# Kotstantinovskiy/SonicDiffusionBayesLab

Measured on AMD Instinct MI355X. Metric: 512x512 images/sec at 50 DDIM steps, higher is better.
Workload: dtype bf16; 1 GPU; SD-1.5 512x512 DDIM 50 steps, CFG 7.5, batch=8/GPU (BASELINE configs[1]); global_batch=8, sample_size=64, parallelism=batch-shard x1, weights=SD-1.5-shaped synthetic seed 1234

## Files before the change

include/sd_hip.h:

```cpp
#ifndef SD_HIP_H
#define SD_HIP_H

#ifdef __cplusplus
extern "C" {
#endif

typedef struct sd_unet sd_unet;

typedef struct sd_unet_config {
    int sample_size;
    int in_channels;
    int out_channels;
    int num_levels;
    int block_out_channels[8];
    int layers_per_block;
    int attn_levels[8];
    int cross_attention_dim;
    int num_heads;
    int norm_num_groups;
    float norm_eps;
    int context_len;
    int weight_dtype;
    float fp8_act_scale_norm;
    float fp8_act_scale_ff;
// ... 65 lines not shown
    int vocab_size;
    int hidden_size;
    int num_layers;
    int num_heads;
    int intermediate_size;
    int max_positions;
    float layer_norm_eps;
} sd_clip_config;
typedef struct sd_unet sd_clip;
int sd_clip_create(const sd_clip_config* cfg, sd_clip** out);
int sd_clip_encode(sd_clip* c, void* stream, const int* input_ids, int batch, float* hidden_out, void* workspace,
                   long long workspace_bytes);

typedef struct sd_clip_vision_config {
    int hidden_size;
    int num_layers;
    int num_heads;
    int intermediate_size;
    int image_size;
    int patch_size;
    int projection_dim;
    float layer_norm_eps;
    int hidden_act;
} sd_clip_vision_config;
enum { SD_ACT_QUICK_GELU = 0, SD_ACT_GELU = 1 };
typedef struct sd_unet sd_clip_vision;
int sd_clip_create_projected(const sd_clip_config* cfg, int projection_dim, int eos_token_id, sd_clip** out);
long long sd_clip_text_embeds_workspace_bytes(sd_clip* c, int batch);
int sd_clip_text_embeds(sd_clip* c, void* stream, const int* input_ids, int batch, float* text_embeds, void* workspace,
                        long long workspace_bytes);
int sd_clip_vision_create(const sd_clip_vision_config* cfg, sd_clip_vision** out);
long long sd_clip_vision_workspace_bytes(sd_clip_vision* v, int batch, int height, int width);
int sd_clip_vision_encode(sd_clip_vision* v, void* stream, const unsigned char* images, int batch, int height, int width,
                          float* image_embeds, void* workspace, long long workspace_bytes);
int sd_clip_score(void* stream, const float* image_embeds, const float* text_embeds, int batch, int dim, float* raw,
                  float* score);
int sd_clip_resize_taps(int in_size, int out_size, int first, int count, int* xmin, int* xcnt, int* coeffs);

typedef struct sd_inception sd_inception;
int sd_inception_create(sd_inception** out);
void sd_inception_destroy(sd_inception* h);
int sd_inception_num_convs(const sd_inception* h);
int sd_inception_conv_info(const sd_inception* h, int index, char* name, int name_cap, long long shape[4]);
int sd_inception_load_conv(sd_inception* h, const char* name, const float* weight_oihw, long long weight_numel,
                           const float* bias, int cout);
int sd_inception_finalize(sd_inception* h);
long long sd_inception_workspace_bytes(sd_inception* h, int batch, int tap);
int sd_inception_features(sd_inception* h, void* stream, const unsigned char* images, int batch, int height, int width,
                          int tap, float* features, void* workspace, long long workspace_bytes);
int sd_fid_accumulate(void* stream, const float* features, int batch, int dim, double* sum, double* cov_sum,
                      long long* count);
int sd_op_inception_conv(void* stream, const void* X, const void* W, const float* bias, void* Y, int B, int Hin, int Win,
                         int Cin, int Cout, int kh, int kw, int stride, int pad_h, int pad_w, int ldy, int coff, int relu);
int sd_op_maxpool3x3(void* stream, const void* X, void* Y, int B, int H, int W, int C, int stride, int pad, int ldy, int coff);
int sd_op_avgpool3x3(void* stream, const void* X, void* Y, int B, int H, int W, int C, int ldy, int coff);
int sd_op_global_mean(void* stream, const void* X, float* out, int B, int HW, int C);
int sd_op_inception_resize(void* stream, const unsigned char* images, int B, int H, int W, void* out, int out_fp32);

#define SD_PROFILE_KINDS 32
int sd_unet_forward_profiled(sd_unet* u, void* stream, const float* latents, int latent_batch, int unet_batch,
                             float timestep, float* eps_out, void* workspace, long long workspace_bytes, int cache_mode,
                             int cache_branch_id, double kind_ms[SD_PROFILE_KINDS], long long kind_launches[SD_PROFILE_KINDS],
                             double kind_flops[SD_PROFILE_KINDS], double kind_bytes[SD_PROFILE_KINDS]);

long long sd_unet_forward_op_times(sd_unet* u, void* stream, const float* latents, int latent_batch, int unet_batch,
                                   float timestep, float* eps_out, void* workspace, long long workspace_bytes, int cache_mode,
                                   int cache_branch_id, char* text, long long cap);

int sd_unet_debug_tensor(sd_unet* u, void* stream, const char* name, float* host_out, long long numel,
                         void* workspace, int unet_batch, int cache_branch_id);

int sd_sched_step(void* stream, const float* eps, int cfg, float guidance, const float* x, const float* m1,
                  const float* m2, const float* m3, const float* noise, float* prev, float* y2, float* m_out,
                  const float coef[10], long long n);

int sd_cfg_rescale_factors(void* stream, const float* eps, int batch, long long n_per_sample, float guidance,
                           float rescale, float* k_out);
int sd_sched_step_rescaled(void* stream, const float* eps, int cfg, float guidance, const float* x, const float* m1,
                           const float* m2, const float* m3, const float* noise, float* prev, float* y2, float* m_out,
                           const float coef[10], long long n, const float* k, long long n_per_sample);

int sd_sched_step_inpaint(void* stream, const float* eps, int cfg, float guidance, const float* x, const float* m1,
                          const float* m2, const float* m3, const float* noise, float* prev, float* y2, float* m_out,
                          const float coef[10], long long n, const float* k, long long n_per_sample, const float* init,
                          const float* blend_noise, const float* mask, float a, float s, long long hw);
int sd_inpaint_prepare(void* stream, const float* image, const float* mask, float* masked_image, float* latent_mask,
                       int batch, int height, int width);

int sd_op_gemm(void* stream, const void* X, long long ldx, const void* X2, long long ldx2, int K1, const void* W,
               const float* bias, const float* bias2, const void* R, long long ldr, void* C, long long ldc, int M,
               int N, int K, int epi);
int sd_op_gemm_tile_rows(int M, int N, int K);
int sd_op_gemm_splitk(int M, int N, int K, int dtype);
int sd_op_gemm_batched(void* stream, const void* X, long long ldx, const void* W, long long w_batch_stride,
                       int rows_per_batch, const float* bias, const void* R, long long ldr, void* C, long long ldc,
                       int M, int N, int K, int epi, int sm_valid);
int sd_op_gemm_batched_softmax_ln(void* stream, const void* X, long long ldx, const void* W, long long w_batch_stride,
                                  int rows_per_batch, void* C, long long ldc, int M, int N, int K, int sm_valid,
                                  const float* rowstats, int parts, const float* c1, const float* c2, float eps);
int sd_op_conv3x3(void* stream, const void* X, const void* W, const float* bias, const float* bias2, const void* R,
                  void* Y, int B, int Hin, int Win, int Cin, int Cout, int stride, int upsample);
int sd_op_conv3x3_shortcut(void* stream, const void* X, const void* W, const float* bias, const void* Xs1, int Cs1,
                           const void* Xs2, int Cs2, const void* Wsc, void* Y, int B, int H, int Wd, int Cin, int Cout);
int sd_op_conv3x3_shortcut_groupnorm(void* stream, const void* X, const void* W, const float* bias, const void* Xs1, int Cs1,
                                     const void* Xs2, int Cs2, const void* Wsc, void* Y, int B, int H, int Wd, int Cin,
                                     int Cout, const float* gamma, const float* beta, void* Yn, int groups, float eps, int silu);
int sd_op_conv3x3_down_asym(void* stream, const void* X, const void* W, const float* bias, void* Y, int B, int Hin, int Win,
                            int Cin, int Cout);
int sd_op_conv3x3_kernel(int M, int N, int Cin, int Hin, int Win, int stride, int upsample, int dtype);
int sd_op_softmax_rows(void* stream, void* S, long long rows, int cols, float scale);
int sd_op_conv3x3_upsample_subpixel(void* stream, const void* X, const void* W4, const float* bias, void* Y, int B, int Hin,
                                    int Win, int Cin, int Cout);
int sd_op_conv3x3_upsample_subpixel_groupnorm(void* stream, const void* X, const void* W4, const float* bias, void* Y, int B,
                                              int Hin, int Win, int Cin, int Cout, const float* gamma, const float* beta,
                                              void* Yn, int groups, float eps, int silu);
int sd_op_groupnorm(void* stream, const void* x1, int C1, const void* x2, int C2, const float* gamma,
                    const float* beta, void* y, int B, int HW, int groups, float eps, int silu);
int sd_op_conv3x3_groupnorm(void* stream, const void* X, const void* W, const float* bias, const float* bias2,
                            const void* R, void* Y, int B, int Hin, int Win, int Cin, int Cout, const float* gamma,
                            const float* beta, void* Yn, int groups, float eps, int silu);
int sd_op_conv3x3_splitk(int M, int Cout, int Cin, int Hin, int Win, int stride, int upsample);
int sd_op_layernorm(void* stream, const void* x, const float* gamma, const float* beta, void* y, int rows, int C,
                    float eps);
int sd_op_attention(void* stream, const void* Q, long long ldq, const void* K, long long ldk, const void* V,
                    long long ldv, void* O, long long ldo, int B, int heads, int Nq, int Nk, int D, float scale);
int sd_op_gemm_qkv_headmajor(void* stream, const void* X, long long ldx, const void* W, void* Q, void* KV, int M, int C,
                             int tokens, int K);
int sd_op_attention_headmajor(void* stream, const void* Q, long long ldq, const void* K, const void* V, void* O,
                              long long ldo, int B, int heads, int Nq, int Nk, int D, float scale);
int sd_op_clip_attention(void* stream, const void* qkv, void* out, int B, int L, int H, int heads);
int sd_op_vit_attention(void* stream, const void* qkv, void* out, int B, int L, int H, int heads);
int sd_op_clip_preprocess(void* stream, const unsigned char* images, int B, int H, int W, int S, int P, unsigned char* crop,
                          void* patches);
int sd_op_conv_in(void* stream, const float* x, int Bsrc, const float* Wt, const float* bias, void* y, int B, int H,
                  int W, int Cin, int Cout);
int sd_op_conv_in_cond(void* stream, const float* x, int Bsrc, const float* cond, int Bcond, const float* Wt,
                       const float* bias, void* y, int B, int H, int W, int Cout);
int sd_op_conv_out(void* stream, const void* x, const void* Wp, const float* bias, float* y, int B, int H, int W,
                   int Cin, int Cout);
int sd_op_time_embedding(void* stream, float t, const void* W1, const float* b1, const void* W2, const float* b2,
                         float* scratch, float* temb, int dim_in, int dim);
int sd_op_timestep_cond(void* stream, float t, const float* cond, const void* Wc, float* row, float* emb, int cond_dim,
                        int dim);

int sd_op_ln_partials(int kind, int M, int N);
int sd_op_gemm_rowstats(void* stream, const void* X, long long ldx, const void* W, const float* bias, const void* R,
                        long long ldr, void* C, long long ldc, int M, int N, int K, float* rowstats);
int sd_op_gemm_ln(void* stream, const void* X, long long ldx, const void* Wg, const float* c1, const float* c2,
                  const float* rowstats, int parts, float eps, void* C, long long ldc, int M, int N, int K, int epi);
int sd_op_gemm_plan(void* stream, const void* X, long long ldx, const void* X2, long long ldx2, int K1, const void* W,
                    const float* bias, const float* bias2, const void* R, long long ldr, void* C, long long ldc, int M, int N,
                    int K, float* rowstats, float* stats, const float* ln_rs, int ln_parts, const float* ln_c1, float ln_eps,
                    void* KV, int hm_tokens);
int sd_op_xattn_fused_rowstats(void* stream, const void* X, const void* R, void* Y, const void* At, const void* Bw,
                               const float* bias, int M, int C, int rows_per_sample, int L, float* rowstats);
int sd_op_ip_xattn(void* stream, const void* R, void* Rout, const void* A, const void* Bt, const float* gamma, const float* beta,
                   float eps, long long M, int C, int rows_per_sample, int heads, int T);
int sd_op_xattn_fused(void* stream, const void* X, const void* R, void* Y, const void* At, const void* Bw,
                      const float* bias, int M, int C, int rows_per_sample, int L);
int sd_op_xattn_fused_ln(void* stream, const void* X, const void* R, void* Y, const void* At, const void* Bw,
                         const float* bias, int M, int C, int rows_per_sample, int L, const float* ln_rowstats, int ln_parts,
                         long long ln_rows, const float* c2, float eps, float* rowstats);
int sd_op_conv3x3_ablate(void* stream, const void* X, const void* W, void* Y, int B, int Hin, int Win, int Cin, int Cout,
                         int ablate);
int sd_op_xattn_fused_stamps(void* stream, const void* X, const void* R, void* Y, const void* At, const void* Bw,
                             const float* bias, int M, int C, int rows_per_sample, int L, unsigned long long* stamps);

int sd_op_gemm_fp8(void* stream, const void* X, long long ldx, const void* W, const float* wscale, float xscale,
                   const float* bias, const void* R, long long ldr, void* C, long long ldc, int M, int N, int K, int epi,
                   int out_fp8, float oscale);
int sd_op_conv3x3_fp8(void* stream, const void* X, const void* W, const float* wscale, float xscale, const float* bias,
                      const float* bias2, const void* R, void* Y, int B, int Hin, int Win, int Cin, int Cout, int stride,
                      int upsample);
int sd_op_groupnorm_fp8(void* stream, const void* x1, int C1, const void* x2, int C2, const float* gamma,
                        const float* beta, void* y, int B, int HW, int groups, float eps, int silu, int Cpad, float oscale);
int sd_op_layernorm_fp8(void* stream, const void* x, const float* gamma, const float* beta, void* y, int rows, int C,
                        int Cpad, float eps, float oscale);
int sd_op_quantize_fp8(void* stream, const void* x_bf16, void* y_fp8, long long rows, int C, int Cpad, float scale);
int sd_op_amax_e4m3(void* stream, const void* codes, long long nbytes, unsigned* out_code);

#ifdef __cplusplus
}
#endif
#endif
```

sonicdiffusionbayeslab_amd/_lib.py:

```python
from __future__ import annotations

import ctypes as C
import os
import re
from typing import Optional

HERE = os.path.dirname(os.path.abspath(__file__))
LIB_PATH = os.environ.get("SD_AMD_LIB", os.path.join(HERE, "lib", "libsdhip.so"))
HEADER_PATH = os.path.normpath(os.path.join(HERE, "..", "include", "sd_hip.h"))

ABLATE_LIB_PATH = os.path.join(HERE, "lib", "libsdhip_ablate.so")

_lib: Optional[C.CDLL] = None
_ablate: Optional[C.CDLL] = None


class SdUnetConfig(C.Structure):
    _fields_ = [
        ("sample_size", C.c_int), ("in_channels", C.c_int), ("out_channels", C.c_int),
        ("num_levels", C.c_int), ("block_out_channels", C.c_int * 8), ("layers_per_block", C.c_int),
        ("attn_levels", C.c_int * 8), ("cross_attention_dim", C.c_int), ("num_heads", C.c_int),
        ("norm_num_groups", C.c_int), ("norm_eps", C.c_float), ("context_len", C.c_int),
        ("weight_dtype", C.c_int), ("fp8_act_scale_norm", C.c_float), ("fp8_act_scale_ff", C.c_float),
        ("time_cond_proj_dim", C.c_int),
        ("ip_adapter_tokens", C.c_int), ("ip_adapter_embed_dim", C.c_int),
    ]


DTYPE_BF16, DTYPE_FP8_E4M3 = 0, 1
DTYPES = {"bf16": DTYPE_BF16, "fp8": DTYPE_FP8_E4M3, "fp8_e4m3": DTYPE_FP8_E4M3}


class SdClipConfig(C.Structure):
    _fields_ = [
        ("vocab_size", C.c_int), ("hidden_size", C.c_int), ("num_layers", C.c_int), ("num_heads", C.c_int),
        ("intermediate_size", C.c_int), ("max_positions", C.c_int), ("layer_norm_eps", C.c_float),
    ]


class SdClipVisionConfig(C.Structure):
    _fields_ = [
        ("hidden_size", C.c_int), ("num_layers", C.c_int), ("num_heads", C.c_int), ("intermediate_size", C.c_int),
        ("image_size", C.c_int), ("patch_size", C.c_int), ("projection_dim", C.c_int), ("layer_norm_eps", C.c_float),
        ("hidden_act", C.c_int),
    ]


class SdHipError(RuntimeError):
    pass


def declared_symbols() -> list:
    src = open(HEADER_PATH).read()
    src = re.sub(r"/\*.*?\*/", "", src, flags=re.S)
    return sorted(set(re.findall(r"\b(sd_[a-z0-9_]+)\s*\(", src)))


_vp, _i, _ll, _f = C.c_void_p, C.c_int, C.c_longlong, C.c_float
_SIGS = {
    "sd_last_error": (C.c_char_p, []),
    "sd_abi_version": (_i, []),
    "sd_unet_create": (_i, [C.POINTER(SdUnetConfig), C.POINTER(_vp)]),
    "sd_unet_destroy": (None, [_vp]),
    "sd_unet_num_params": (_i, [_vp]),
    "sd_unet_param_info": (_i, [_vp, _i, C.c_char_p, _i, C.POINTER(_ll), C.POINTER(_i)]),
    "sd_unet_load_param": (_i, [_vp, C.c_char_p, _vp, _ll]),
    "sd_unet_finalize": (_i, [_vp]),
    "sd_unet_debug_packed": (_ll, [_vp, C.c_char_p, _vp, _ll]),
    "sd_unet_calibrate_fp8": (_i, [_vp, _vp, _vp, _i, _i, _f, _f, _vp, _ll]),
    "sd_unet_fp8_scale_count": (_i, [_vp]),
    "sd_unet_fp8_scale_info": (_i, [_vp, _i, C.c_char_p, _i, C.POINTER(_f), C.POINTER(_f)]),
    "sd_unet_set_fp8_scale": (_i, [_vp, C.c_char_p, _f]),
    "sd_unet_workspace_bytes": (_ll, [_vp, _i, _i]),
    "sd_unet_set_context": (_i, [_vp, _vp, _vp, _i, _i, _vp, _ll]),
    "sd_unet_set_timestep_cond": (_i, [_vp, _vp, _vp]),
    "sd_unet_forward": (_i, [_vp, _vp, _vp, _i, _i, _f, _vp, _vp, _ll, _i, _i]),
    "sd_unet_workspace_bytes_hw": (_ll, [_vp, _i, _i, _i, _i]),
    "sd_unet_set_context_hw": (_i, [_vp, _vp, _vp, _i, _i, _i, _i, _vp, _ll]),
    "sd_unet_forward_hw": (_i, [_vp, _vp, _vp, _i, _i, _i, _i, _f, _vp, _vp, _ll, _i, _i]),
    "sd_unet_forward_profiled": (_i, [_vp, _vp, _vp, _i, _i, _f, _vp, _vp, _ll, _i, _i, C.POINTER(C.c_double),
                                      C.POINTER(_ll), C.POINTER(C.c_double), C.POINTER(C.c_double)]),
    "sd_unet_forward_op_times": (_ll, [_vp, _vp, _vp, _i, _i, _f, _vp, _vp, _ll, _i, _i, C.c_char_p, _ll]),
    "sd_vae_create": (_i, [C.POINTER(SdUnetConfig), C.POINTER(_vp)]),
    "sd_vae_decode": (_i, [_vp, _vp, _vp, _i, _f, _vp, _vp, _ll]),
    "sd_vae_decode_hw": (_i, [_vp, _vp, _vp, _i, _i, _i, _f, _vp, _vp, _ll]),
    "sd_vae_encoder_create": (_i, [C.POINTER(SdUnetConfig), C.POINTER(_vp)]),
    "sd_vae_encode_hw": (_i, [_vp, _vp, _vp, _i, _i, _i, _vp, _vp, _ll]),
    "sd_vae_posterior_sample": (_i, [_vp, _vp, _vp, _f, _vp, _i, _ll]),
    "sd_clip_create": (_i, [C.POINTER(SdClipConfig), C.POINTER(_vp)]),
    "sd_clip_encode": (_i, [_vp, _vp, _vp, _i, _vp, _vp, _ll]),
    "sd_clip_create_projected": (_i, [C.POINTER(SdClipConfig), _i, _i, C.POINTER(_vp)]),
    "sd_clip_text_embeds_workspace_bytes": (_ll, [_vp, _i]),
    "sd_clip_text_embeds": (_i, [_vp, _vp, _vp, _i, _vp, _vp, _ll]),
    "sd_clip_vision_create": (_i, [C.POINTER(SdClipVisionConfig), C.POINTER(_vp)]),
    "sd_clip_vision_workspace_bytes": (_ll, [_vp, _i, _i, _i]),
    "sd_clip_vision_encode": (_i, [_vp, _vp, _vp, _i, _i, _i, _vp, _vp, _ll]),
    "sd_clip_score": (_i, [_vp, _vp, _vp, _i, _i, _vp, _vp]),
    "sd_clip_resize_taps": (_i, [_i, _i, _i, _i, _vp, _vp, _vp]),
    "sd_op_vit_attention": (_i, [_vp, _vp, _vp, _i, _i, _i, _i]),
    "sd_op_clip_preprocess": (_i, [_vp, _vp, _i, _i, _i, _i, _i, _vp, _vp]),
    "sd_inception_create": (_i, [C.POINTER(_vp)]),
    "sd_inception_destroy": (None, [_vp]),
    "sd_inception_num_convs": (_i, [_vp]),
    "sd_inception_conv_info": (_i, [_vp, _i, C.c_char_p, _i, C.POINTER(_ll)]),
    "sd_inception_load_conv": (_i, [_vp, C.c_char_p, _vp, _ll, _vp, _i]),
    "sd_inception_finalize": (_i, [_vp]),
    "sd_inception_workspace_bytes": (_ll, [_vp, _i, _i]),
    "sd_inception_features": (_i, [_vp, _vp, _vp, _i, _i, _i, _i, _vp, _vp, _ll]),
    "sd_fid_accumulate": (_i, [_vp, _vp, _i, _i, _vp, _vp, _vp]),
    "sd_op_inception_conv": (_i, [_vp, _vp, _vp, _vp, _vp, _i, _i, _i, _i, _i, _i, _i, _i, _i, _i, _i, _i, _i]),
    "sd_op_maxpool3x3": (_i, [_vp, _vp, _vp, _i, _i, _i, _i, _i, _i, _i, _i]),
    "sd_op_avgpool3x3": (_i, [_vp, _vp, _vp, _i, _i, _i, _i, _i, _i]),
    "sd_op_global_mean": (_i, [_vp, _vp, _vp, _i, _i, _i]),
    "sd_op_inception_resize": (_i, [_vp, _vp, _i, _i, _i, _vp, _i]),
    "sd_unet_debug_tensor": (_i, [_vp, _vp, C.c_char_p, _vp, _ll, _vp, _i, _i]),
    "sd_sched_step": (_i, [_vp, _vp, _i, _f, _vp, _vp, _vp, _vp, _vp, _vp, _vp, _vp, C.POINTER(_f), _ll]),
    "sd_cfg_rescale_factors": (_i, [_vp, _vp, _i, _ll, _f, _f, _vp]),
    "sd_sched_step_rescaled": (_i, [_vp, _vp, _i, _f, _vp, _vp, _vp, _vp, _vp, _vp, _vp, _vp, C.POINTER(_f), _ll, _vp, _ll]),
    "sd_sched_step_inpaint": (_i, [_vp, _vp, _i, _f, _vp, _vp, _vp, _vp, _vp, _vp, _vp, _vp, C.POINTER(_f), _ll, _vp, _ll,
                                   _vp, _vp, _vp, _f, _f, _ll]),
    "sd_inpaint_prepare": (_i, [_vp, _vp, _vp, _vp, _vp, _i, _i, _i]),
    "sd_unet_set_inpaint_cond_hw": (_i, [_vp, _vp, _vp, _vp, _i, _i, _i]),
    "sd_unet_set_ip_adapter_hw": (_i, [_vp, _vp, _vp, _i, _i, _i, _i, _f, _vp, _ll]),
    "sd_op_ip_xattn": (_i, [_vp, _vp, _vp, _vp, _vp, _vp, _vp, _f, _ll, _i, _i, _i, _i]),
    "sd_op_conv_in_cond": (_i, [_vp, _vp, _i, _vp, _i, _vp, _vp, _vp, _i, _i, _i, _i]),
    "sd_op_gemm": (_i, [_vp, _vp, _ll, _vp, _ll, _i, _vp, _vp, _vp, _vp, _ll, _vp, _ll, _i, _i, _i, _i]),
    "sd_op_gemm_tile_rows": (_i, [_i, _i, _i]),
    "sd_op_gemm_splitk": (_i, [_i, _i, _i, _i]),
    "sd_op_gemm_batched": (_i, [_vp, _vp, _ll, _vp, _ll, _i, _vp, _vp, _ll, _vp, _ll, _i, _i, _i, _i, _i]),
    "sd_op_gemm_batched_softmax_ln": (_i, [_vp, _vp, _ll, _vp, _ll, _i, _vp, _ll, _i, _i, _i, _i, _vp, _i, _vp, _vp, _f]),
    "sd_op_conv3x3": (_i, [_vp, _vp, _vp, _vp, _vp, _vp, _vp, _i, _i, _i, _i, _i, _i, _i]),
    "sd_op_conv3x3_shortcut": (_i, [_vp, _vp, _vp, _vp, _vp, _i, _vp, _i, _vp, _vp, _i, _i, _i, _i, _i]),
    "sd_op_conv3x3_shortcut_groupnorm": (_i, [_vp, _vp, _vp, _vp, _vp, _i, _vp, _i, _vp, _vp, _i, _i, _i, _i, _i,
                                              _vp, _vp, _vp, _i, _f, _i]),
    "sd_op_conv3x3_down_asym": (_i, [_vp, _vp, _vp, _vp, _vp, _i, _i, _i, _i, _i]),
    "sd_op_conv3x3_ablate": (_i, [_vp, _vp, _vp, _vp, _i, _i, _i, _i, _i, _i]),
    "sd_op_conv3x3_upsample_subpixel": (_i, [_vp, _vp, _vp, _vp, _vp, _i, _i, _i, _i, _i]),
    "sd_op_conv3x3_upsample_subpixel_groupnorm": (_i, [_vp, _vp, _vp, _vp, _vp, _i, _i, _i, _i, _i, _vp, _vp, _vp, _i, _f, _i]),
    "sd_op_groupnorm": (_i, [_vp, _vp, _i, _vp, _i, _vp, _vp, _vp, _i, _i, _i, _f, _i]),
    "sd_op_conv3x3_groupnorm": (_i, [_vp, _vp, _vp, _vp, _vp, _vp, _vp, _i, _i, _i, _i, _i, _vp, _vp, _vp, _i, _f, _i]),
    "sd_op_conv3x3_splitk": (_i, [_i, _i, _i, _i, _i, _i, _i]),
    "sd_op_conv3x3_kernel": (_i, [_i, _i, _i, _i, _i, _i, _i, _i]),
    "sd_op_softmax_rows": (_i, [_vp, _vp, _ll, _i, _f]),
    "sd_op_layernorm": (_i, [_vp, _vp, _vp, _vp, _vp, _i, _i, _f]),
    "sd_op_attention": (_i, [_vp, _vp, _ll, _vp, _ll, _vp, _ll, _vp, _ll, _i, _i, _i, _i, _i, _f]),
    "sd_op_gemm_qkv_headmajor": (_i, [_vp, _vp, _ll, _vp, _vp, _vp, _i, _i, _i, _i]),
    "sd_op_attention_headmajor": (_i, [_vp, _vp, _ll, _vp, _vp, _vp, _ll, _i, _i, _i, _i, _i, _f]),
    "sd_op_clip_attention": (_i, [_vp, _vp, _vp, _i, _i, _i, _i]),
    "sd_op_conv_in": (_i, [_vp, _vp, _i, _vp, _vp, _vp, _i, _i, _i, _i, _i]),
    "sd_op_conv_out": (_i, [_vp, _vp, _vp, _vp, _vp, _i, _i, _i, _i, _i]),
    "sd_op_time_embedding": (_i, [_vp, _f, _vp, _vp, _vp, _vp, _vp, _vp, _i, _i]),
    "sd_op_timestep_cond": (_i, [_vp, _f, _vp, _vp, _vp, _vp, _i, _i]),
    "sd_op_ln_partials": (_i, [_i, _i, _i]),
    "sd_op_gemm_rowstats": (_i, [_vp, _vp, _ll, _vp, _vp, _vp, _ll, _vp, _ll, _i, _i, _i, _vp]),
    "sd_op_gemm_plan": (_i, [_vp, _vp, _ll, _vp, _ll, _i, _vp, _vp, _vp, _vp, _ll, _vp, _ll, _i, _i, _i, _vp, _vp, _vp, _i, _vp, _f,
                            _vp, _i]),
    "sd_op_gemm_ln": (_i, [_vp, _vp, _ll, _vp, _vp, _vp, _vp, _i, _f, _vp, _ll, _i, _i, _i, _i]),
    "sd_op_xattn_fused_rowstats": (_i, [_vp, _vp, _vp, _vp, _vp, _vp, _vp, _i, _i, _i, _i, _vp]),
    "sd_op_xattn_fused": (_i, [_vp, _vp, _vp, _vp, _vp, _vp, _vp, _i, _i, _i, _i]),
    "sd_op_xattn_fused_ln": (_i, [_vp, _vp, _vp, _vp, _vp, _vp, _vp, _i, _i, _i, _i, _vp, _i, _ll, _vp, _f, _vp]),
    "sd_op_xattn_fused_stamps": (_i, [_vp, _vp, _vp, _vp, _vp, _vp, _vp, _i, _i, _i, _i, _vp]),
    "sd_op_gemm_fp8": (_i, [_vp, _vp, _ll, _vp, _vp, _f, _vp, _vp, _ll, _vp, _ll, _i, _i, _i, _i, _i, _f]),
    "sd_op_conv3x3_fp8": (_i, [_vp, _vp, _vp, _vp, _f, _vp, _vp, _vp, _vp, _i, _i, _i, _i, _i, _i, _i]),
    "sd_op_groupnorm_fp8": (_i, [_vp, _vp, _i, _vp, _i, _vp, _vp, _vp, _i, _i, _i, _f, _i, _i, _f]),
    "sd_op_layernorm_fp8": (_i, [_vp, _vp, _vp, _vp, _vp, _i, _i, _i, _f, _f]),
    "sd_op_quantize_fp8": (_i, [_vp, _vp, _vp, _ll, _i, _i, _f]),
    "sd_op_amax_e4m3": (_i, [_vp, _vp, _ll, _vp]),
}


def load() -> C.CDLL:
    global _lib
    if _lib is not None:
        return _lib
    if not os.path.exists(LIB_PATH):
        raise SdHipError(
            f"{LIB_PATH} is missing: build it with `python -m sonicdiffusionbayeslab_amd.build` "
            "(or __graft_entry__.build()).  There is no CPU/PyTorch fallback for the hot path.")
    lib = C.CDLL(LIB_PATH)
    for name, (res, args) in _SIGS.items():
        fn = getattr(lib, name)
        fn.restype = res
        fn.argtypes = args
    _lib = lib
    return lib


def load_ablate() -> C.CDLL:
    global _ablate
    if _ablate is not None:
        return _ablate
    if not os.path.exists(ABLATE_LIB_PATH):
        raise SdHipError(f"{ABLATE_LIB_PATH} is missing: build it with `python -m sonicdiffusionbayeslab_amd.build`")
    lib = C.CDLL(ABLATE_LIB_PATH)
    for name, (res, args) in _SIGS.items():
        fn = getattr(lib, name)
        fn.restype = res
        fn.argtypes = args
    _ablate = lib
    return lib


def check(rc: int, what: str = "libsdhip call", lib: Optional[C.CDLL] = None) -> None:
    if rc != 0:
        msg = (lib or load()).sd_last_error()
        raise SdHipError(f"{what} failed (rc={rc}): {msg.decode() if msg else '?'}")


def ptr(t) -> Optional[int]:
    return None if t is None else t.data_ptr()


def current_stream() -> int:
    import torch
    return torch.cuda.current_stream().cuda_stream
```

sonicdiffusionbayeslab_amd/csrc/conv_halo.hip:

```cpp
#include "common.h"
#include "kernels.h"

#include <stdlib.h>

#include <algorithm>

namespace {

constexpr int BM = 256, BN = 160;
constexpr int TN = 5, WTN = 80;
constexpr int HSLOTS = 400;
constexpr int HBYTES = HSLOTS * 128;
constexpr int WPIECES = BN / 8;
constexpr int WBYTES = WPIECES * 1024;
constexpr int WSTAGES = 3;
constexpr int SMEM = 2 * HBYTES + WSTAGES * WBYTES;
static_assert(SMEM <= 160 * 1024, "halo tile does not fit the 160 KiB LDS");
constexpr unsigned NOSRC = 0xffffffffu;

template <int N>
__device__ __forceinline__ void wait_vmcnt() {
    asm volatile("s_waitcnt vmcnt(%0)" ::"n"(N) : "memory");
}

__device__ __forceinline__ int swz_of(int row, int dt) { return dt ? (((row >> 1) & 1) | (row & 4)) : (row & 7); }

template <int DT, int DIAG = 0, int NWV = 8, int SUB = 0, int GEN = 0, int SC = 0>
__global__ __launch_bounds__(NWV * 64, NWV == 8 ? 2 : 1) void conv_halo_kernel(const GemmArgs p) {
    static_assert(NWV == 8 || (NWV == 4 && DT == 0), "4-wave layout: bf16 only");
    static_assert(!SC || (DT == 0 && DIAG == 0 && NWV == 8 && SUB == 0), "shortcut phase: bf16, 8 waves, 9 taps");
    static_assert(!SUB || (DT == 0 && DIAG == 0 && NWV == 8), "sub-pixel upsampler: bf16, 8 waves");
    static_assert(!GEN || (SUB == 0 && DIAG == 0 && NWV == 8), "geometry mode: 9 taps, 8 waves");
    constexpr int NTAP = SUB ? 4 : 9;
    constexpr int NT = NWV * 64;
    constexpr int WMW = NWV == 8 ? 4 : 2;
    constexpr int TM = BM / WMW / 16, WTM = TM * 16;
    constexpr int HPIECES = NWV == 8 ? 7 : 13;
    constexpr int WPW = NWV == 8 ? 3 : 5;
    constexpr bool CARRY = NWV == 4;
    constexpr int ESZ = DT ? 1 : 2;
    extern __shared__ __attribute__((aligned(16))) char smem[];
    const int tid = threadIdx.x, lane = tid & 63;
    const int wave = __builtin_amdgcn_readfirstlane(tid >> 6);

    int work = blockIdx.x;
    {
        const int nblk = gridDim.x;
        const int q = nblk >> 3, r = nblk & 7, xcd = work & 7, idx = work >> 3;
        work = (xcd < r ? xcd * (q + 1) : r * (q + 1) + (xcd - r) * q) + idx;
    }
    const int ntiles = p.tiles_m * p.tiles_n;
    const int nwork = ntiles * (SUB ? 4 : p.splitk);
    if (work >= nwork) return;
    const int S = (p.Cin * ESZ) >> 7;
    const int Mrows = SUB ? p.M >> 2 : p.M;

    const int up = SUB ? 0 : p.up;
    const int Ho = SUB ? p.Hin : p.Hout, Wo = SUB ? p.Win : p.Wout, HWo = Ho * Wo;
    const int RW = GEN ? p.rows_per_batch : min(Ho, BM / Wo);
    const int PW = p.Win + 2, PP = ((RW >> up) + 2) * PW;
    const int PIX = RW * Wo;
    const int HP = GEN ? PP : (BM / PIX) * PP;
    const int tpi = GEN ? (Ho + RW - 1) / RW : 1;

    const char* Xb = (const char*)p.X;
    const char* Wg = (const char*)p.W;

    constexpr int HREL_ZERO = (int)0x80000000;
    const int lgW = __builtin_ctz(Wo), lgHW = __builtin_ctz(HWo);
    const int RWin = RW >> up;
    int hrel[HPIECES];
    int hyv[GEN ? HPIECES : 1];
    const int jdup = wave < 2 ? HPIECES - 1 : HPIECES - 2;
#pragma unroll
    for (int j = 0; j < HPIECES; ++j) {
        const int L = (j == HPIECES - 1 ? jdup : j) * NT + tid;
        const int slot = L >> 3, cpos = L & 7;
        const int i = slot / PP, rem = slot - i * PP;
        const int hy = rem / PW, hx = rem - hy * PW;
        const bool ok = slot < HP && hx >= 1 && hx <= p.Win;
        hrel[j] = ok ? ((((hy - 1) * p.Win + (hx - 1)) * p.Cin * ESZ + ((cpos ^ swz_of(slot, DT)) << 4)) | i |
                        (hy == 0 ? 4 : 0) | (hy == RWin + 1 ? 8 : 0))
                     : HREL_ZERO;
        if (GEN) hyv[j] = hy;
    }

    auto wpiece = [&](int i) { return NWV == 4 ? wave + 4 * i : (i < 2 ? wave + 8 * i : (wave < 4 ? wave + 16 : wave + 8)); };

    int split = 0, m0 = 0, n0 = 0, s_begin = 0, s_end = 0, phase = 0;
    int mend = 0;
    unsigned hoff[HPIECES];
    unsigned woffs[WPW];
    auto setup = [&](int w) {
        int tile_n, tile_m;
        if (SUB) {
            const int C = 4 * p.tiles_n, rect = (p.tiles_m >> 3) * (C >> 2) * 32;
            const bool rects = gridDim.x == 256 && p.tune == 0;
            int combo;
            if (rects && w < rect) {
                const int r = w >> 5, i = w & 31, bc = r % (C >> 2);
                tile_m = (r / (C >> 2)) * 8 + (i >> 2);
                combo = bc * 4 + (i & 3);
            } else {
                const int w2 = rects ? w - rect : w;
                tile_m = (rects ? (p.tiles_m & ~7) : 0) + w2 / C;
                combo = w2 % C;
            }
            tile_n = combo % p.tiles_n;
            phase = combo / p.tiles_n;
            split = 0; s_begin = 0; s_end = S;
        } else {
            split = w / ntiles;
            const int t = w - split * ntiles;
            tile_n = t % p.tiles_n, tile_m = t / p.tiles_n;
            s_begin = (int)((long)S * split / p.splitk);
            s_end = (int)((long)S * (split + 1) / p.splitk);
        }
        m0 = tile_m * BM;
        n0 = tile_n * BN;
        if (GEN) {
            const int b = tile_m / tpi, y0 = (tile_m - b * tpi) * RW;
            m0 = b * HWo + y0 * Wo;
            mend = m0 + min(RW, Ho - y0) * Wo;
            const int ybase = y0 >> up;
            const unsigned base = (unsigned)(((long)b * p.Hin + ybase) * p.Win * p.Cin * ESZ);
#pragma unroll
            for (int j = 0; j < HPIECES; ++j) {
                const int iy = ybase - 1 + hyv[j];
                const bool ok = hrel[j] != HREL_ZERO && iy >= 0 && iy < p.Hin;
                hoff[j] = ok ? base + (unsigned)(hrel[j] & ~15) : NOSRC;
            }
        } else {
#pragma unroll
        for (int j = 0; j < HPIECES; ++j) {
            const int mp = m0 + (hrel[j] & 3) * PIX;
            const int b = mp >> lgHW;
            const int ybase = (mp & (HWo - 1)) >> (lgW + up);
            const bool ok = hrel[j] != HREL_ZERO && mp < Mrows && !((hrel[j] & 4) && ybase == 0) &&
                            !((hrel[j] & 8) && ybase + RWin == p.Hin);
            const unsigned base = (unsigned)(((long)b * p.Hin + ybase) * p.Win * p.Cin * ESZ);
            hoff[j] = ok ? base + (unsigned)(hrel[j] & ~15) : NOSRC;
        }
        }
#pragma unroll
        for (int i = 0; i < WPW; ++i) {
            const int pc = wpiece(i);
            const int n = n0 + pc * 8 + (lane >> 3);
            const int c = (lane & 7) ^ swz_of(lane >> 3, DT);
            woffs[i] = n < p.N ? (unsigned)(((SUB ? (long)phase * p.w_batch_stride : 0l) + (long)n * p.ldw) * ESZ + (c << 4)) : NOSRC;
        }
    };
    const unsigned xbytes = (unsigned)((long)(Mrows / HWo) * p.Hin * p.Win * p.Cin * ESZ);
    const unsigned wbytes = (unsigned)((long)p.N * p.ldw * ESZ * (SUB ? 4 : 1));
    auto issue_h = [&](int j, int s, char* hb) {
        const __amdgpu_buffer_rsrc_t r = __builtin_amdgcn_make_buffer_rsrc((void*)Xb, 0, (int)(s >= 0 ? xbytes : 0u), 0x00020000);
        __builtin_amdgcn_raw_ptr_buffer_load_lds(r, LDS_PTR(hb + ((j == HPIECES - 1 ? jdup : j) * NWV + wave) * 1024), 16, (int)hoff[j],
                                                 s >= 0 ? s * 128 : 0, 0, 0);
    };
    auto issue_w1 = [&](int i, int kk, char* wb) {
        const __amdgpu_buffer_rsrc_t r = __builtin_amdgcn_make_buffer_rsrc((void*)Wg, 0, (int)(kk >= 0 ? wbytes : 0u), 0x00020000);
        __builtin_amdgcn_raw_ptr_buffer_load_lds(r, LDS_PTR(wb + wpiece(i) * 1024), 16, (int)woffs[i], kk >= 0 ? kk * 128 : 0, 0, 0);
    };
    auto issue_h_tap = [&](int tap, int s, char* hb) {
        if (SUB) {
            if (tap < 3) {
                issue_h(2 * tap, s, hb);
                issue_h(2 * tap + 1, s, hb);
            } else {
                issue_h(6, s, hb);
            }
        } else if (NWV == 8) {
            if (tap < 7) issue_h(tap, s, hb);
        } else if (tap < 5) {
            issue_h(2 * tap, s, hb);
            issue_h(2 * tap + 1, s, hb);
        } else if (tap < 8) {
            issue_h(tap + 5, s, hb);
        }
    };
    auto issue_w = [&](int kk, char* wb) {
#pragma unroll
        for (int i = 0; i < WPW; ++i) issue_w1(i, kk, wb);
    };

    const int wm = wave % WMW, wn = wave / WMW;
    const int lrow = lane & 15, lq = lane >> 4;
    int hbase[TM], hrc[TM];
#pragma unroll
    for (int f = 0; f < TM; ++f) {
        if (GEN) {
            const int pt = min(wm * WTM + f * 16 + lrow, PIX - 1);
            const int row = pt / Wo;
            hrc[f] = row << 16 | (pt - row * Wo);
            hbase[f] = PW + 1;
        } else {
        const int pt = wm * WTM + f * 16 + lrow;
        const int i = pt / PIX, rem = pt - i * PIX;
        hrc[f] = (rem >> lgW) << 16 | (rem & (Wo - 1));
        hbase[f] = i * PP + PW + 1;
        }
    }
    const int wfrag = (wn * WTN + lrow) * 128;
    const int wswz0 = DT ? ((2 * lq) ^ swz_of(lane, 1)) << 4 : (lq ^ (lane & 7)) << 4;

    const int sc_gch = ((lane & 7) ^ (lane >> 3)) << 4;
    const int scp1 = SC ? p.Csc1 * 2 : 0, scp2 = SC ? p.Csc2 * 2 : 0, scpw = SC ? (int)p.ldwsc * 2 : 0;
    const int vXs1 = (lane >> 3) * scp1 + sc_gch, vXs2 = (lane >> 3) * scp2 + sc_gch, vWs = (lane >> 3) * scpw + sc_gch;
    const int scfrag = (wm * WTM + lrow) * 128 + ((lq ^ (lane & 7)) << 4);

    auto frag_addr = [&](int f, int tp) -> int {
        const int hp = hbase[f] + (((hrc[f] >> 16) + (tp / 3 - 1)) >> up) * PW + (((hrc[f] & 0xffff) + (tp % 3 - 1)) >> up);
        return hp * 128 + (DT ? (((2 * lq) ^ swz_of(hp, 1)) << 4) : ((lq ^ (hp & 7)) << 4));
    };

    auto frag_addr_sub = [&](int f, int t) -> int {
        const int hp = hbase[f] + ((hrc[f] >> 16) + (phase >> 1) + (t >> 1) - 1) * PW + ((hrc[f] & 0xffff) + (phase & 1) + (t & 1) - 1);
        return hp * 128 + ((lq ^ (hp & 7)) << 4);
    };

    f32x4 acc[TN][TM];
    bf16x8 xf0[TM], wf0[TN], xf1[TM], wf1[TN];
    int xan[TM];
#pragma unroll
    for (int f = 0; f < TM; ++f) xan[f] = frag_addr(f, 0);
    auto mfmas = [&](const bf16x8* xf, const bf16x8* wf) {
#pragma unroll
        for (int a = 0; a < TN; ++a)
#pragma unroll
            for (int b = 0; b < TM; ++b)
                acc[a][b] = __builtin_amdgcn_mfma_f32_16x16x32_bf16(wf[a], xf[b], acc[a][b], 0, 0, 0);
    };
    i32x8 wq[DT ? TN : 1], xq[2];
    auto ld32 = [&](const char* base, int off) -> i32x8 {
        return cat_u32x4(*(const u32x4*)(base + off), *(const u32x4*)(base + (off ^ 16)));
    };

    char* const Hb0 = smem;
    char* const Hb1 = smem + HBYTES;
    char* const Wb = smem + 2 * HBYTES;

    int hsel = 0, wst = 0;
    setup(work);
#pragma unroll
    for (int j = 0; j < HPIECES; ++j) issue_h(j, s_begin, Hb0);
    issue_w(s_begin * NTAP, Wb);
    issue_w(s_begin * NTAP + 1, Wb + WBYTES);
    bool stores_pending = false;
    constexpr int FULL_STORES = (TN / 2 + TN % 2) * TM;

    while (true) {
#pragma unroll
        for (int a = 0; a < TN; ++a)
#pragma unroll
            for (int b = 0; b < TM; ++b) acc[a][b] = f32x4{0.f, 0.f, 0.f, 0.f};
        if (CARRY) {
#pragma unroll
            for (int f = 0; f < TM; ++f) xf1[f] = bf16x8{0, 0, 0, 0, 0, 0, 0, 0};
#pragma unroll
            for (int a = 0; a < TN; ++a) wf1[a] = bf16x8{0, 0, 0, 0, 0, 0, 0, 0};
        }

        for (int s = s_begin; s < s_end; ++s) {
            const char* hcur = hsel ? Hb1 : Hb0;
            char* hnext = hsel ? Hb0 : Hb1;
            const bool more = s + 1 < s_end;
            if (DT || NWV == 4) {
#pragma unroll
                for (int f = 0; f < TM; ++f) asm volatile("" : "+v"(hbase[f]), "+v"(hrc[f]));
            }
#pragma unroll
            for (int tap = 0; tap < NTAP; ++tap) {
                if (SUB) {
                    if (tap == 0) {
                        if (s == s_begin && stores_pending) wait_vmcnt<3 + FULL_STORES>();
                        else wait_vmcnt<3>();
                    } else {
                        wait_vmcnt<5>();
                    }
                } else if (DIAG == 0) {
                if (NWV == 8) {
                if (tap == 0) {
                    if (s == s_begin && stores_pending) wait_vmcnt<3 + FULL_STORES>();
                    else wait_vmcnt<3>();
                } else if (tap == 8) {
                    wait_vmcnt<3>();
                } else {
                    wait_vmcnt<4>();
                }
                } else {
                if (tap == 0) {
                    if (s == s_begin && stores_pending) wait_vmcnt<5 + FULL_STORES>();
                    else wait_vmcnt<5>();
                } else if (tap <= 5) {
                    wait_vmcnt<7>();
                } else {
                    wait_vmcnt<6>();
                }
                }
                }
                if (!(DIAG & 4)) __builtin_amdgcn_s_barrier();
                asm volatile("" ::: "memory");
                const char* wcur = Wb + wst * WBYTES;
                char* wnext = Wb + (wst == 0 ? 2 : wst - 1) * WBYTES;
                int xa[TM];
#pragma unroll
                for (int f = 0; f < TM; ++f) xa[f] = CARRY ? xan[f] : SUB ? frag_addr_sub(f, tap) : frag_addr(f, tap);
                if (CARRY) {
                    if (!(DIAG & 8) || (tap == 0 && s == s_begin)) {
#pragma unroll
                    for (int f = 0; f < TM; ++f) xf0[f] = *(const bf16x8*)(hcur + xa[f]);
#pragma unroll
                    for (int a = 0; a < TN; ++a) wf0[a] = *(const bf16x8*)(wcur + wfrag + a * 2048 + wswz0);
                    }
                    if ((DIAG & 8) && tap == 0 && s == s_begin) {
#pragma unroll
                        for (int f = 0; f < TM; ++f) xf1[f] = xf0[f];
#pragma unroll
                        for (int a = 0; a < TN; ++a) wf1[a] = wf0[a];
                    }
                    __builtin_amdgcn_sched_barrier(0);
                    const int hs = more ? s + 1 : -1, kw = s * 9 + tap + 2 < s_end * 9 ? s * 9 + tap + 2 : -1;
#pragma unroll
                    for (int a = 0; a < TN; ++a) {
#pragma unroll
                        for (int b = 0; b < TM; ++b) {
                            acc[a][b] = __builtin_amdgcn_mfma_f32_16x16x32_bf16(wf1[a], xf1[b], acc[a][b], 0, 0, 0);
                            const int idx = a * TM + b;
                            if (idx % 5 == 4 && !(DIAG & 2)) {
                                const int pc = idx / 5;
                                if (pc < WPW) issue_w1(pc, kw, wnext);
                                else if (tap < 5 && pc < WPW + 2) issue_h(2 * tap + (pc - WPW), hs, hnext);
                                else if (tap < 8 && pc == WPW) issue_h(tap + 5, hs, hnext);
                            }
                        }
                    }
                    __builtin_amdgcn_sched_barrier(0);
                    if (!(DIAG & 8)) {
#pragma unroll
                    for (int f = 0; f < TM; ++f) xf1[f] = *(const bf16x8*)(hcur + (xa[f] ^ 64));
#pragma unroll
                    for (int a = 0; a < TN; ++a) wf1[a] = *(const bf16x8*)(wcur + wfrag + a * 2048 + (wswz0 ^ 64));
                    }
#pragma unroll
                    for (int f = 0; f < TM; ++f) xan[f] = frag_addr(f, tap == 8 ? 0 : tap + 1);
                    mfmas(xf0, wf0);
                    __builtin_amdgcn_sched_barrier(0);
                    __builtin_amdgcn_s_waitcnt(0xc07f);
                } else if (DT) {
#pragma unroll
                    for (int a = 0; a < TN; ++a) wq[a] = ld32(wcur, wfrag + a * 2048 + wswz0);
                    xq[0] = ld32(hcur, xa[0]);
                    __builtin_amdgcn_sched_barrier(0);
                    issue_h_tap(tap, more ? s + 1 : -1, hnext);
                    issue_w(s * 9 + tap + 2 < s_end * 9 ? s * 9 + tap + 2 : -1, wnext);
                    __builtin_amdgcn_sched_barrier(0);
#pragma unroll
                    for (int b = 0; b < TM; ++b) {
                        if (b + 1 < TM) xq[(b + 1) & 1] = ld32(hcur, xa[b + 1]);
#pragma unroll
                        for (int a = 0; a < TN; ++a)
                            acc[a][b] = __builtin_amdgcn_mfma_scale_f32_16x16x128_f8f6f4(wq[a], xq[b & 1], acc[a][b], 0, 0, 0, 0, 0, 0);
                    }
                } else {
                    if (!(DIAG & 8)) {
#pragma unroll
                    for (int f = 0; f < TM; ++f) xf0[f] = *(const bf16x8*)(hcur + xa[f]);
#pragma unroll
                    for (int a = 0; a < TN; ++a) wf0[a] = *(const bf16x8*)(wcur + wfrag + a * 2048 + wswz0);
                    }
                    __builtin_amdgcn_sched_barrier(0);
                    if (!(DIAG & 2)) {
                    issue_h_tap(tap, more ? s + 1 : -1, hnext);
                    issue_w(s * NTAP + tap + 2 < s_end * NTAP ? s * NTAP + tap + 2 : -1, wnext);
                    }
                    __builtin_amdgcn_sched_barrier(0);
                    if (!(DIAG & 8)) {
#pragma unroll
                    for (int f = 0; f < TM; ++f) xf1[f] = *(const bf16x8*)(hcur + (xa[f] ^ 64));
#pragma unroll
                    for (int a = 0; a < TN; ++a) wf1[a] = *(const bf16x8*)(wcur + wfrag + a * 2048 + (wswz0 ^ 64));
                    } else if (tap == 0 && s == s_begin) {
#pragma unroll
                        for (int f = 0; f < TM; ++f) xf0[f] = xf1[f] = *(const bf16x8*)(hcur + xa[f]);
#pragma unroll
                        for (int a = 0; a < TN; ++a) wf0[a] = wf1[a] = *(const bf16x8*)(wcur + wfrag + a * 2048 + wswz0);
                    }
                    mfmas(xf0, wf0);
                    mfmas(xf1, wf1);
                }
                wst = wst == 2 ? 0 : wst + 1;
            }
            hsel ^= 1;
        }
        if (CARRY) mfmas(xf1, wf1);

        if (SC) {
            const int nsc = (p.Csc1 + p.Csc2) >> 6, nsc1 = p.Csc1 >> 6;
            const int t_begin = (int)((long)nsc * split / p.splitk), t_end = (int)((long)nsc * (split + 1) / p.splitk);
            if (t_begin < t_end) {
                const unsigned rows = (unsigned)(GEN ? min(mend, p.M) : p.M);
                auto stage_sc = [&](int t, char* xb, char* wb) {
                    const bool seg1 = t < nsc1;
                    const int pitch = seg1 ? scp1 : scp2;
                    const __amdgpu_buffer_rsrc_t rx = __builtin_amdgcn_make_buffer_rsrc((void*)(seg1 ? p.Xs1 : p.Xs2), 0,
                                                                                        (int)(rows * (unsigned)pitch), 0x00020000);
                    const int vx = seg1 ? vXs1 : vXs2;
                    const int so = (m0 + wave * 8) * pitch + (seg1 ? t : t - nsc1) * 128;
#pragma unroll
                    for (int i = 0; i < BM / 64; ++i)
                        __builtin_amdgcn_raw_ptr_buffer_load_lds(rx, LDS_PTR(xb + (wave + 8 * i) * 1024), 16, vx, so + i * 64 * pitch, 0, 0);
                    const __amdgpu_buffer_rsrc_t rw = __builtin_amdgcn_make_buffer_rsrc((void*)p.Wsc, 0, (int)((unsigned)p.N * (unsigned)scpw), 0x00020000);
#pragma unroll
                    for (int i = 0; i < WPW; ++i) {
                        const int pc = wpiece(i);
                        __builtin_amdgcn_raw_ptr_buffer_load_lds(rw, LDS_PTR(wb + pc * 1024), 16, vWs, (n0 + pc * 8) * scpw + t * 128, 0, 0);
                    }
                };
                char* const xlast = hsel ? Hb0 : Hb1;
                char* const xprev = hsel ? Hb1 : Hb0;
                char* const wlast = Wb + (wst == 0 ? 2 : wst - 1) * WBYTES;
                char* const wprev = Wb + wst * WBYTES;
                wait_vmcnt<0>();
                __builtin_amdgcn_s_barrier();
                asm volatile("" ::: "memory");
                {
                    const bool e0 = ((t_end - 1 - t_begin) & 1) == 0;
                    stage_sc(t_begin, e0 ? xlast : xprev, e0 ? wlast : wprev);
                }
                for (int t = t_begin; t < t_end; ++t) {
                    const bool e = ((t_end - 1 - t) & 1) == 0;
                    const char* xcur = e ? xlast : xprev;
                    const char* wcur = e ? wlast : wprev;
                    wait_vmcnt<0>();
                    __builtin_amdgcn_s_barrier();
                    asm volatile("" ::: "memory");
#pragma unroll
                    for (int f = 0; f < TM; ++f) xf0[f] = *(const bf16x8*)(xcur + scfrag + f * 2048);
#pragma unroll
                    for (int a = 0; a < TN; ++a) wf0[a] = *(const bf16x8*)(wcur + wfrag + a * 2048 + wswz0);
                    __builtin_amdgcn_sched_barrier(0);
                    if (t + 1 < t_end) stage_sc(t + 1, e ? xprev : xlast, e ? wprev : wlast);
                    __builtin_amdgcn_sched_barrier(0);
#pragma unroll
                    for (int f = 0; f < TM; ++f) xf1[f] = *(const bf16x8*)(xcur + ((scfrag + f * 2048) ^ 64));
#pragma unroll
                    for (int a = 0; a < TN; ++a) wf1[a] = *(const bf16x8*)(wcur + wfrag + a * 2048 + (wswz0 ^ 64));
                    mfmas(xf0, wf0);
                    mfmas(xf1, wf1);
                }
            }
        }

        const int em0 = m0, en0 = n0, esplit = split, ephase = phase;
        const int elim = GEN ? mend : Mrows;
        auto crow = [&](int m) -> long {
            if (!SUB) return m;
            const int b = m >> lgHW, ml = m & (HWo - 1);
            return ((long)b * p.Hout + 2 * (ml >> lgW) + (ephase >> 1)) * p.Wout + 2 * (ml & (Wo - 1)) + (ephase & 1);
        };
        if (DT && p.splitk == 1) {
#pragma unroll
            for (int a = 0; a < TN; ++a) {
                const int n = min(en0 + wn * WTN + a * 16 + lq * 4, p.N - 4);
                const f32x4 sv = *(const f32x4*)(p.wscale + n) * p.xscale_inv;
#pragma unroll
                for (int b = 0; b < TM; ++b) acc[a][b] *= sv;
            }
        }
        if (p.splitk == 1) {
            if (SC == 0 && p.R) {
                u32x2 rr[TN][TM];
#pragma unroll
                for (int a = 0; a < TN; ++a) {
                    const int n = min(en0 + wn * WTN + a * 16 + lq * 4, p.N - 4);
#pragma unroll
                    for (int b = 0; b < TM; ++b) {
                        const int m = min(em0 + wm * WTM + b * 16 + lrow, elim - 1);
                        rr[a][b] = *(const u32x2*)(p.R + crow(m) * p.ldr + n);
                    }
                }
#pragma unroll
                for (int a = 0; a < TN; ++a)
#pragma unroll
                    for (int b = 0; b < TM; ++b) {
                        acc[a][b][0] += bflo(rr[a][b][0]); acc[a][b][1] += bfhi(rr[a][b][0]);
                        acc[a][b][2] += bflo(rr[a][b][1]); acc[a][b][3] += bfhi(rr[a][b][1]);
                    }
            }
            if (p.bias) {
#pragma unroll
                for (int a = 0; a < TN; ++a) {
                    const int n = min(en0 + wn * WTN + a * 16 + lq * 4, p.N - 4);
                    f32x4 bv = *(const f32x4*)(p.bias + n);
                    if (SC == 0 && p.bias2) bv += *(const f32x4*)(p.bias2 + n);
#pragma unroll
                    for (int b = 0; b < TM; ++b) acc[a][b] += bv;
                }
            }
        }

        work += gridDim.x;
        const bool more_work = work < nwork;
        const bool wide_ok = (p.ldc & 7) == 0;
        if (more_work) {
            setup(work);
            wait_vmcnt<0>();
            char* hb = hsel ? Hb1 : Hb0;
#pragma unroll
            for (int j = 0; j < HPIECES; ++j) issue_h(j, s_begin, hb);
            issue_w(s_begin * NTAP, Wb + wst * WBYTES);
            issue_w(s_begin * NTAP + 1, Wb + (wst == 2 ? 0 : wst + 1) * WBYTES);
            stores_pending = p.splitk == 1 && wide_ok && (em0 + BM <= elim) && (en0 + BN <= p.N);
        }

        if (p.splitk > 1) {
            float* slab = p.slab + (long)esplit * p.M * p.N;
#pragma unroll
            for (int a = 0; a < TN; ++a) {
                const int n = en0 + wn * WTN + a * 16 + lq * 4;
                if (n >= p.N) continue;
#pragma unroll
                for (int b = 0; b < TM; ++b) {
                    const int m = em0 + wm * WTM + b * 16 + lrow;
                    if (m >= (GEN ? elim : p.M)) continue;
                    *(f32x4*)(slab + (long)m * p.N + n) = acc[a][b];
                }
            }
        } else {
            if (!GEN && p.stats) {
                const int r0 = em0 + wm * WTM;
                const int blk0 = SUB ? ((((r0 >> lgHW) << 2) + ephase) << (lgHW - 6)) + ((r0 & (HWo - 1)) >> 6) : r0 >> 6;
#pragma unroll
                for (int hb64 = 0; hb64 < TM / 4; ++hb64)
                    tile_channel_stats<TN, TM>(acc, p.stats, blk0 + hb64, p.N, en0 + wn * WTN, p.N,
                                               em0 + wm * WTM, Mrows, lane, 4 * hb64, 4);
            }
            auto store_narrow = [&](int a) {
                const int n = en0 + wn * WTN + a * 16 + lq * 4;
                if (n >= p.N) return;
#pragma unroll
                for (int b = 0; b < TM; ++b) {
                    const int m = em0 + wm * WTM + b * 16 + lrow;
                    const f32x4 v = acc[a][b];
                    u32x2 o = {pack2bf(v[0], v[1]), pack2bf(v[2], v[3])};
                    if (m < elim) *(u32x2*)(p.C + crow(m) * p.ldc + n) = o;
                }
            };
#pragma unroll
            for (int a = 0; a < TN; a += 2) {
                const int nb = en0 + wn * WTN + a * 16;
                if (a + 1 < TN && wide_ok && nb + 32 <= p.N) {
#pragma unroll
                    for (int b = 0; b < TM; ++b) {
                        const int m = em0 + wm * WTM + b * 16 + lrow;
                        const f32x4 vx = acc[a][b], vy = acc[a + 1 < TN ? a + 1 : a][b];
                        const auto s0 = __builtin_amdgcn_permlane16_swap(pack2bf(vx[0], vx[1]), pack2bf(vy[0], vy[1]), false, false);
                        const auto s1 = __builtin_amdgcn_permlane16_swap(pack2bf(vx[2], vx[3]), pack2bf(vy[2], vy[3]), false, false);
                        const u32x4 o = {s0[0], s1[0], s0[1], s1[1]};
                        const int col = nb + (lq & 1) * 16 + (lq >> 1) * 8;
                        if (m < elim) *(u32x4*)(p.C + crow(m) * p.ldc + col) = o;
                    }
                } else {
                    store_narrow(a);
                    if (a + 1 < TN) store_narrow(a + 1);
                }
            }
        }
        if (!more_work) break;
    }
}

bool halo_enabled() {
    static const char* env = getenv("SD_CONV_HALO");
    return env ? atoi(env) != 0 : true;
}

}

static bool pow2_applicable(const GemmArgs& a);
static int launch_halo_gen(GemmArgs a, hipStream_t stream);

bool sd_conv_halo_applicable(const GemmArgs& a) {
    return sd_conv_halo_mode(a) != 0;
}

static int gen_rows(const GemmArgs& a) {
    const int H = a.Hin << a.up, W = a.Win << a.up;
    if (W < 8 || W > BM) return 0;
    int rw = std::min(H, BM / W);
    if (a.up) rw &= ~1;
    while (rw > 0 && ((rw >> a.up) + 2) * (a.Win + 2) > HSLOTS) rw -= a.up ? 2 : 1;
    return rw;
}

int sd_conv_halo_mode(const GemmArgs& a) {
    if (!halo_enabled() || a.stride != 1) return 0;
    const long ldw0 = a.ldw ? a.ldw : a.K;
    if ((long)a.M * a.Cin * 2 >= (1l << 32) || (long)a.N * ldw0 * 2 >= (1l << 32)) return 0;
    if (a.dt == 1 && a.Cin % 128) return 0;
    if (pow2_applicable(a)) return 1;
    const char* env = getenv("SD_CONV_HALO_GEN");
    if ((env && atoi(env) == 0) || a.subpix || a.stats) return 0;
    const int H = a.Hin << a.up, W = a.Win << a.up;
    if (a.M % (H * W)) return 0;
    const int rw = gen_rows(a);
    return rw > 0 && rw * W >= 192 ? 2 : 0;
}

static bool pow2_applicable(const GemmArgs& a) {
    if (!halo_enabled() || a.stride != 1) return false;
    const int H = a.Hin << a.up, W = a.Win << a.up;
    if (W < 8 || W > BM || BM % W) return false;
    const int RW = H < BM / W ? H : BM / W;
    const int PIX = RW * W;
    if (BM % PIX || (H * W) % PIX || (a.up && (RW & 1))) return false;
    if ((W & (W - 1)) || ((H * W) & (H * W - 1))) return false;
    if ((BM / PIX) * ((RW >> a.up) + 2) * (a.Win + 2) > HSLOTS) return false;
    const long ldw = a.ldw ? a.ldw : a.K;
    if ((long)a.M * a.Cin * 2 >= (1l << 32) || (long)a.N * ldw * 2 >= (1l << 32)) return false;
    if (a.dt == 1 && a.Cin % 128) return false;
    return true;
}

bool sd_conv_halo_shortcut_applicable(const GemmArgs& a) {
    if (a.dt != 0 || a.subpix || a.up || a.stride != 1 || a.R != nullptr || a.bias2 != nullptr || a.tune != 0) return false;
    if (!sd_conv_halo_applicable(a)) return false;
    if (a.Csc1 < 64 || a.Csc1 % 64 || a.Csc2 < 0 || a.Csc2 % 64) return false;
    const long ldw = a.ldwsc ? a.ldwsc : a.Csc1 + a.Csc2;
    if (ldw < a.Csc1 + a.Csc2 || (ldw & 7)) return false;
    const long big = 1l << 32;
    return ((long)a.M + BM) * std::max(a.Csc1, a.Csc2) * 2 < big && ((long)a.N + BN) * ldw * 2 < big;
}

bool sd_conv_halo_subpix_applicable(const GemmArgs& a) {
    const char* env = getenv("SD_SUBPIX_HALO");
    const bool off = env && atoi(env) == 0;
    if (off || !a.subpix || a.dt != 0 || a.R != nullptr || (a.splitk > 1 && a.slab) || (a.Hin * a.Win) % 64 != 0) return false;
    GemmArgs g = a;
    g.up = 0; g.stride = 1; g.M = a.M / 4;
    if (!sd_conv_halo_applicable(g)) return false;
    const long ldw = a.ldw ? a.ldw : a.K;
    if ((long)a.N * 4 * ldw * 2 >= (1l << 32)) return false;
    if (a.w_batch_stride != (long)a.N * ldw) return false;
    return (long)((g.M + BM - 1) / BM) * 4 * ((a.N + BN - 1) / BN) >= 256;
}

int sd_conv_halo_splitk(int M, int N, int Cin, int dt) {
    const int tiles = ((M + BM - 1) / BM) * ((N + BN - 1) / BN);
    if (tiles >= 192) return 1;
    const int S = Cin / (dt ? 128 : 64);
    int want = (256 + tiles - 1) / tiles;
    int maxs = tiles < 64 ? S / 2 : S / 4;
    int s = want < maxs ? want : maxs;
    if (s > 8) s = 8;
    return s < 1 ? 1 : s;
}

int sd_conv3x3_splitk(int M, int N, int Cin, int Hin, int Win, int stride, int up, int dt) {
    static const char* env = getenv("SD_SPLITK");
    GemmArgs a;
    a.M = M; a.N = N; a.Cin = Cin; a.K = 9 * Cin; a.ldw = a.K; a.Hin = Hin; a.Win = Win; a.stride = stride; a.up = up; a.dt = dt;
    if (!env && sd_conv_halo_applicable(a)) return sd_conv_halo_splitk(M, N, Cin, dt);
    return sd_gemm_splitk(M, N, dt ? 9 * Cin / 2 : 9 * Cin, 128);
}

int sd_launch_conv3x3_halo(const GemmArgs& a0, hipStream_t stream) {
    GemmArgs a = a0;
    a.tiles_m = ((a.subpix ? a.M / 4 : a.M) + BM - 1) / BM;
    a.tiles_n = (a.N + BN - 1) / BN;
    if (a.ldw == 0) a.ldw = a.K;
    if (a.slab == nullptr || a.splitk < 1) a.splitk = 1;
    SD_REQUIRE(!a.defer_reduce || a.splitk > 1, "conv3x3 halo: defer_reduce needs split-K (the consumer would read an unwritten slab)");
    if (a.subpix) {
        SD_REQUIRE(a.dt == 0 && a.splitk == 1 && a.R == nullptr && a.up == 0 && a.K == 4 * a.Cin && a.w_batch_stride > 0 &&
                       a.Hout == 2 * a.Hin && a.Wout == 2 * a.Win && a.M % (4 * a.Hin * a.Win) == 0 && a0.tune == 0,
                   "conv3x3 halo, sub-pixel upsampler: bf16, no split-K, no residual, K = 4 Cin");
        SD_REQUIRE(a.w_batch_stride == (long)a.N * a.ldw, "conv3x3 halo, sub-pixel upsampler: phase stride %ld != N * ldw = %ld",
                   a.w_batch_stride, (long)a.N * a.ldw);
        static bool sub_attr_set = false;
        if (!sub_attr_set) {
            SD_CHECK_HIP(hipFuncSetAttribute((const void*)conv_halo_kernel<0, 0, 8, 1>, hipFuncAttributeMaxDynamicSharedMemorySize, SMEM));
            sub_attr_set = true;
        }
        int g = a.tiles_m * a.tiles_n * 4;
        if (g > 256) g = 256;
        static const bool old_order = getenv("SD_SUBPIX_ORDER") && atoi(getenv("SD_SUBPIX_ORDER")) == 0;
        a.tune = old_order ? 1 : 0;
        hipLaunchKernelGGL((conv_halo_kernel<0, 0, 8, 1>), dim3(g), dim3(512), SMEM, stream, a);
        SD_CHECK_HIP(hipGetLastError());
        return 0;
    }
    const int slices = a.Cin / (a.dt ? 128 : 64);
    SD_REQUIRE(a.splitk <= slices, "conv3x3 halo: splitk %d exceeds the %d channel slices", a.splitk, slices);
    if (a.Wsc) {
        SD_REQUIRE(a.Xs1 && (a.Xs2 || a.Csc2 == 0) && sd_conv_halo_shortcut_applicable(a0),
                   "conv3x3 halo: the 1x1 shortcut (%d + %d channels) cannot ride on this conv", a.Csc1, a.Csc2);
        if (a.ldwsc == 0) a.ldwsc = a.Csc1 + a.Csc2;
        if (a.Csc2 == 0) a.Xs2 = a.Xs1;
    }
    if (!pow2_applicable(a0)) return launch_halo_gen(a, stream);
    static bool attr_set = false;
    if (!attr_set) {
        SD_CHECK_HIP(hipFuncSetAttribute((const void*)conv_halo_kernel<0>, hipFuncAttributeMaxDynamicSharedMemorySize, SMEM));
        SD_CHECK_HIP(hipFuncSetAttribute((const void*)conv_halo_kernel<1>, hipFuncAttributeMaxDynamicSharedMemorySize, SMEM));
        SD_CHECK_HIP(hipFuncSetAttribute((const void*)conv_halo_kernel<0, 0, 8, 0, 0, 1>, hipFuncAttributeMaxDynamicSharedMemorySize, SMEM));
#ifdef SD_ABLATE
        SD_CHECK_HIP(hipFuncSetAttribute((const void*)conv_halo_kernel<0, 1>, hipFuncAttributeMaxDynamicSharedMemorySize, SMEM));
        SD_CHECK_HIP(hipFuncSetAttribute((const void*)conv_halo_kernel<0, 3>, hipFuncAttributeMaxDynamicSharedMemorySize, SMEM));
        SD_CHECK_HIP(hipFuncSetAttribute((const void*)conv_halo_kernel<0, 7>, hipFuncAttributeMaxDynamicSharedMemorySize, SMEM));
        SD_CHECK_HIP(hipFuncSetAttribute((const void*)conv_halo_kernel<0, 15>, hipFuncAttributeMaxDynamicSharedMemorySize, SMEM));
        SD_CHECK_HIP(hipFuncSetAttribute((const void*)conv_halo_kernel<0, 0, 4>, hipFuncAttributeMaxDynamicSharedMemorySize, SMEM));
        SD_CHECK_HIP(hipFuncSetAttribute((const void*)conv_halo_kernel<0, 15, 4>, hipFuncAttributeMaxDynamicSharedMemorySize, SMEM));
#endif
        attr_set = true;
    }
    int grid = a.tiles_m * a.tiles_n * a.splitk;
    if (grid > 256) grid = 256;
    if (a.Wsc) {
        a.tune = 0;
        hipLaunchKernelGGL((conv_halo_kernel<0, 0, 8, 0, 0, 1>), dim3(grid), dim3(512), SMEM, stream, a);
        if (a.splitk > 1 && !a.defer_reduce) sd_launch_splitk_reduce(a, stream);
        SD_CHECK_HIP(hipGetLastError());
        return 0;
    }
#ifdef SD_ABLATE
    const int tune = a0.tune;
    a.tune = tune;
    static const int env_waves = getenv("SD_CONV_WAVES") ? atoi(getenv("SD_CONV_WAVES")) : 8;
    const int waves = (tune & 256) ? 4 : env_waves;
    if (a.dt) hipLaunchKernelGGL(conv_halo_kernel<1>, dim3(grid), dim3(512), SMEM, stream, a);
    else if (waves == 4 && (tune & 15) == 8) hipLaunchKernelGGL((conv_halo_kernel<0, 15, 4>), dim3(grid), dim3(256), SMEM, stream, a);
    else if (waves == 4 && (tune & 15) == 0) hipLaunchKernelGGL((conv_halo_kernel<0, 0, 4>), dim3(grid), dim3(256), SMEM, stream, a);
    else if ((tune & 15) == 1) hipLaunchKernelGGL((conv_halo_kernel<0, 1>), dim3(grid), dim3(512), SMEM, stream, a);
    else if ((tune & 15) == 2) hipLaunchKernelGGL((conv_halo_kernel<0, 3>), dim3(grid), dim3(512), SMEM, stream, a);
    else if ((tune & 15) == 4) hipLaunchKernelGGL((conv_halo_kernel<0, 7>), dim3(grid), dim3(512), SMEM, stream, a);
    else if ((tune & 15) == 8) hipLaunchKernelGGL((conv_halo_kernel<0, 15>), dim3(grid), dim3(512), SMEM, stream, a);
    else hipLaunchKernelGGL(conv_halo_kernel<0>, dim3(grid), dim3(512), SMEM, stream, a);
#else
    SD_REQUIRE(a0.tune == 0, "conv3x3 (halo): this build carries no ablation kernels (load libsdhip_ablate.so)");
    a.tune = 0;
    if (a.dt) hipLaunchKernelGGL(conv_halo_kernel<1>, dim3(grid), dim3(512), SMEM, stream, a);
    else hipLaunchKernelGGL(conv_halo_kernel<0>, dim3(grid), dim3(512), SMEM, stream, a);
#endif
    if (a.splitk > 1 && !a.defer_reduce) sd_launch_splitk_reduce(a, stream);
    SD_CHECK_HIP(hipGetLastError());
    return 0;
}

static int launch_halo_gen(GemmArgs a, hipStream_t stream) {
    const int Ho = a.Hin << a.up, Wo = a.Win << a.up, rw = gen_rows(a);
    SD_REQUIRE(rw > 0 && a.Hout == Ho && a.Wout == Wo && a.M % (Ho * Wo) == 0 && !a.stats && a.tune == 0,
               "conv3x3 halo (geometry mode): shape %dx%d -> %dx%d not taken", a.Hin, a.Win, Ho, Wo);
    a.rows_per_batch = rw;
    a.tiles_m = (a.M / (Ho * Wo)) * ((Ho + rw - 1) / rw);
    static bool attr_set = false;
    if (!attr_set) {
        SD_CHECK_HIP(hipFuncSetAttribute((const void*)conv_halo_kernel<0, 0, 8, 0, 1>, hipFuncAttributeMaxDynamicSharedMemorySize, SMEM));
        SD_CHECK_HIP(hipFuncSetAttribute((const void*)conv_halo_kernel<1, 0, 8, 0, 1>, hipFuncAttributeMaxDynamicSharedMemorySize, SMEM));
        SD_CHECK_HIP(hipFuncSetAttribute((const void*)conv_halo_kernel<0, 0, 8, 0, 1, 1>, hipFuncAttributeMaxDynamicSharedMemorySize, SMEM));
        attr_set = true;
    }
    int grid = a.tiles_m * a.tiles_n * a.splitk;
    if (grid > 256) grid = 256;
    if (a.Wsc) hipLaunchKernelGGL((conv_halo_kernel<0, 0, 8, 0, 1, 1>), dim3(grid), dim3(512), SMEM, stream, a);
    else if (a.dt) hipLaunchKernelGGL((conv_halo_kernel<1, 0, 8, 0, 1>), dim3(grid), dim3(512), SMEM, stream, a);
    else hipLaunchKernelGGL((conv_halo_kernel<0, 0, 8, 0, 1>), dim3(grid), dim3(512), SMEM, stream, a);
    if (a.splitk > 1 && !a.defer_reduce) sd_launch_splitk_reduce(a, stream);
    SD_CHECK_HIP(hipGetLastError());
    return 0;
}
```

sonicdiffusionbayeslab_amd/csrc/kernels.h:

```cpp
#pragma once
#include <vector>

#include "common.h"

struct GemmArgs {
    const bf16_t* X = nullptr;
    long ldx = 0;
    const bf16_t* X2 = nullptr;
    long ldx2 = 0;
    int K1 = 0;
    const bf16_t* W = nullptr;
    long ldw = 0;
    const float* bias = nullptr;
    const float* bias2 = nullptr;
    const bf16_t* R = nullptr;
    long ldr = 0;
    bf16_t* C = nullptr;
    long ldc = 0;
    int M = 0, N = 0, K = 0;
    int Hin = 0, Win = 0, Cin = 0, Hout = 0, Wout = 0, stride = 1, up = 0;
    int asym = 0;
    int splitk = 1;
    float* slab = nullptr;
    int defer_reduce = 0;
    const void* zero_page = nullptr;
    long w_batch_stride = 0;
    int rows_per_batch = 0;
    int sm_valid = 0;
    int tiles_m = 0, tiles_n = 0;
    int tune = 0;
    float* stats = nullptr;
    float* rowstats = nullptr;
    bf16_t* KV = nullptr;
    int hm_C = 0, hm_tok = 0;
    int subpix = 0;
    const float* ln_rs = nullptr;
    const float* ln_c1 = nullptr;
    int ln_np = 0;
    float ln_eps = 1e-5f;
    int ln_per_sample = 0;
    int dt = 0;
    const float* wscale = nullptr;
    float xscale_inv = 1.0f;
    int out_fp8 = 0;
    float oscale = 1.0f;
    const bf16_t* Xs1 = nullptr;
    const bf16_t* Xs2 = nullptr;
    const bf16_t* Wsc = nullptr;
    long ldwsc = 0;
    int Csc1 = 0, Csc2 = 0;
};

int sd_gemm_tile_rows(int M, int N, int K = 0);
int sd_gemm_splitk(int M, int N, int K, int rows = 0);
int sd_launch_gemm(const GemmArgs& a, int epi , hipStream_t stream);
int sd_launch_conv3x3(const GemmArgs& a, hipStream_t stream);
bool sd_gemm_lean_applicable(const GemmArgs& a, int epi);
int sd_launch_gemm_lean(const GemmArgs& a, int epi, int rows, hipStream_t stream);
void sd_launch_splitk_reduce(const GemmArgs& a, hipStream_t stream);
bool sd_conv_halo_applicable(const GemmArgs& a);
int sd_conv_halo_mode(const GemmArgs& a);
int sd_conv3x3_splitk(int M, int N, int Cin, int Hin, int Win, int stride, int up, int dt = 0);
bool sd_conv_halo_subpix_applicable(const GemmArgs& a);
int sd_launch_conv3x3_halo(const GemmArgs& a, hipStream_t stream);
bool sd_conv_halo_shortcut_applicable(const GemmArgs& a);

struct GroupNormArgs {
    const bf16_t* x1 = nullptr; int C1 = 0;
    const bf16_t* x2 = nullptr; int C2 = 0;
    const float* gamma = nullptr; const float* beta = nullptr;
    bf16_t* y = nullptr;
    int out_fp8 = 0, Cpad = 0;
    float oscale = 1.0f;
    const float* stats1 = nullptr; const float* stats2 = nullptr;
    const float* slab = nullptr; int splitk = 0;
    const float* sbias = nullptr; const float* sbias2 = nullptr;
    const bf16_t* sR = nullptr; long sldr = 0;
    bf16_t* x1w = nullptr;
    float* partial = nullptr;
    int B = 0, HW = 0, groups = 32, nsplit = 0;
    float eps = 1e-5f;
    int silu = 0;
};
int sd_groupnorm_nsplit(int B, int HW);
bool sd_groupnorm_uses_small(int B, int HW, int C1, int C2, int groups);
bool sd_groupnorm_slab_ok(int B, int HW, int C1, int C2, int groups);
size_t sd_groupnorm_scratch_bytes(int B, int HW, int groups);
int sd_launch_groupnorm(const GroupNormArgs& a, hipStream_t stream);

int sd_launch_softmax_rows(bf16_t* s, long rows, int cols, float scale, hipStream_t stream);
int sd_launch_softmax_rows_long(bf16_t* s, long rows, int cols, float scale, hipStream_t stream);
int sd_launch_pqconv(const float* x, const float* W, const float* bias, float* y, int B, int HW, float in_scale,
                     hipStream_t stream);

int sd_launch_layernorm(const bf16_t* x, const float* gamma, const float* beta, bf16_t* y, int rows, int C,
                        float eps, hipStream_t stream);
int sd_launch_layernorm_fp8(const bf16_t* x, const float* gamma, const float* beta, void* y, int rows, int C, int Cpad,
                            float eps, float oscale, hipStream_t stream);
int sd_launch_amax_e4m3(const void* y, long nbytes, unsigned* out, hipStream_t stream);
int sd_launch_quantize_fp8(const bf16_t* x, void* y, long rows, int C, int Cpad, float scale, hipStream_t stream);

struct AttnArgs {
    const bf16_t* Q = nullptr; long ldq = 0;
    const bf16_t* K = nullptr; long ldk = 0;
    const bf16_t* V = nullptr; long ldv = 0;
    bf16_t* O = nullptr; long ldo = 0;
    int B = 0, heads = 0, Nq = 0, Nk = 0, D = 0;
    float scale = 0.f;
    const void* consts = nullptr;
    int kv_head_major = 0;
    int q_prescaled = 0;
    int xcd_order = 1;
};
int sd_launch_attention(const AttnArgs& a, hipStream_t stream);

int sd_launch_gemv(const float* x, const bf16_t* W, const float* b, float* y, int N, int K, int silu_in,
                   hipStream_t stream);
int sd_launch_timestep_sinusoid(float t, float* out, int dim, hipStream_t stream);
int sd_launch_timestep_sinusoid_row(float t, const float* row, float* out, int dim, hipStream_t stream);
int sd_launch_f32_to_bf16(const float* src, bf16_t* dst, long n, hipStream_t stream);
int sd_launch_transpose_bf16(const bf16_t* src, bf16_t* dst, int B, int R, int Cc, hipStream_t stream, int perm16 = 0);

int sd_launch_retile32(const bf16_t* src, bf16_t* dst, int B, int R, int K, int RT, hipStream_t stream);
int sd_launch_replicate(const void* src, void* dst, long bytes, int rep, hipStream_t stream);

struct XattnArgs {
    const bf16_t* X = nullptr;
    const bf16_t* R = nullptr;
    bf16_t* Y = nullptr;
    const bf16_t* At = nullptr;
    const bf16_t* Bw = nullptr;
    const float* bias = nullptr;
    int M = 0, C = 0, rows_per_sample = 0, L = 0;
    float* rowstats = nullptr;
    const float* ln_rs = nullptr; int ln_np = 0; long ln_rows = 0;
    const float* ln_c2 = nullptr;
    float ln_eps = 1e-5f;
    unsigned long long* stamps = nullptr;
};
bool sd_xattn_fused_applicable(int rows_per_sample, int C, int heads, int L);
int sd_xattn_slices(int M, int C);
int sd_launch_xattn_fused(const XattnArgs& a, hipStream_t stream);
int sd_launch_xattn_expand(const bf16_t* kv, bf16_t* out, int B, int L, int C, int NH, int col_off, float scale,
                           hipStream_t stream, int slots = 80);
bool sd_ip_xattn_applicable(int C, int heads, int T);
int sd_launch_ip_xattn(const bf16_t* R, bf16_t* Y, const bf16_t* A, const bf16_t* Bt, const float* gamma, const float* beta,
                       float eps, long M, int C, int rows_per_sample, int heads, int T, hipStream_t stream);
int sd_launch_clip_embed(const int* ids, const bf16_t* tok, const bf16_t* pos, bf16_t* out, int rows, int L, int H,
                         int vocab, hipStream_t stream);
int sd_launch_clip_attention(const bf16_t* qkv, bf16_t* out, int B, int L, int H, int heads, hipStream_t stream);
int sd_launch_quick_gelu(bf16_t* x, long n, hipStream_t stream);
int sd_launch_gelu_erf(bf16_t* x, long n, hipStream_t stream);
int sd_launch_bf16_to_f32(const bf16_t* src, float* dst, long n, hipStream_t stream);

struct ClipPrepGeom {
    int H = 0, W = 0, S = 0, y0 = 0, R = 0, ksx = 0, ksy = 0;
    int o_xmin = 0, o_xcnt = 0, o_xk = 0, o_ymin = 0, o_ycnt = 0, o_yk = 0;
};
void sd_clip_resize_geometry(int H, int W, int S, int* rh, int* rw, int* top, int* left);
int sd_clip_prep_tables(int H, int W, int S, std::vector<int>& tab, ClipPrepGeom& g);
int sd_launch_clip_preprocess(const unsigned char* img, int B, const ClipPrepGeom& g, const int* dtab, unsigned char* tmp,
                              bf16_t* patches, int P, int Kp, unsigned char* crop, hipStream_t stream);
int sd_launch_vit_embed(const bf16_t* prow, const float* cls, const bf16_t* pos, bf16_t* out, int B, int Np, int H,
                        hipStream_t stream);
int sd_launch_vit_attention(const bf16_t* qkv, bf16_t* out, int B, int L, int H, int heads, hipStream_t stream);
int sd_launch_pool_rows(const bf16_t* src, const int* ids, int B, int L, int H, int eos_id, bf16_t* dst, hipStream_t stream);
int sd_launch_clip_score(const float* img, const float* txt, int B, int P, float* raw, float* score, hipStream_t stream);

int sd_launch_conv_in(const float* x, int Bsrc, const float* Wt , const float* bias,
                      bf16_t* y, int B, int H, int W, int Cin, int Cout, hipStream_t stream);
int sd_launch_conv_in_cond(const float* x, int Bsrc, const float* cond, int Bcond, const float* Wt, const float* bias,
                           bf16_t* y, int B, int H, int W, int Cout, hipStream_t stream);
int sd_launch_inpaint_cond_pack(const float* mask, const float* masked, float* cond, int B, long hw, hipStream_t stream);
int sd_launch_inpaint_prepare(const float* img, const float* mask, float* masked, float* lmask, int B, int H, int W,
                              hipStream_t stream);
int sd_launch_conv_in_image(const float* img, const float* Wt , const float* bias, bf16_t* y, int B, int H,
                            int W, int Cout, hipStream_t stream);
int sd_launch_vae_enc_out(const bf16_t* x, const bf16_t* Wp , const float* bias, const float* Wq ,
                          const float* bq, float* y, int B, int H, int W, int Cin, hipStream_t stream);
int sd_launch_vae_posterior(const float* moments, const float* noise, float scale, float* z, int B, int C, long hw,
                            hipStream_t stream);
int sd_launch_conv_out(const bf16_t* x, const bf16_t* Wp , const float* bias, float* y, int B,
                       int H, int W, int Cin, int Cout, hipStream_t stream);

struct StepCoef {
    float px, pe, p1, p2, pn;
    float yx, ye;
    float mx, me;
    float p3;
};
int sd_launch_sched_step(const float* eps, int cfg, float guidance, const float* x, const float* m1,
                         const float* m2, const float* m3, const float* noise, float* prev, float* y2, float* m_out,
                         StepCoef c, long n, hipStream_t stream);
int sd_launch_cfg_rescale_factors(const float* eps, int batch, long n_per_sample, float guidance, float rescale, float* k_out,
                                  hipStream_t stream);
int sd_launch_sched_step_rescaled(const float* eps, int cfg, float guidance, const float* x, const float* m1,
                                  const float* m2, const float* m3, const float* noise, float* prev, float* y2,
                                  float* m_out, StepCoef c, const float* k, long n_per_sample, long n, hipStream_t stream);
int sd_launch_sched_step_inpaint(const float* eps, int cfg, float guidance, const float* x, const float* m1,
                                 const float* m2, const float* m3, const float* noise, float* prev, float* y2,
                                 float* m_out, StepCoef c, const float* k, long n_per_sample, long n, const float* init,
                                 const float* blend_noise, const float* mask, float a, float s, long hw, hipStream_t stream);

int sd_launch_inception_conv(const bf16_t* x, const bf16_t* w, const float* bias, bf16_t* y, int B, int Hin, int Win, int Cin,
                             int Cout, int kh, int kw, int stride, int ph, int pw, int ldy, int coff, int relu,
                             hipStream_t stream);
int sd_launch_inception_pool(const bf16_t* x, bf16_t* y, int B, int H, int W, int C, int stride, int pad, int avg, int ldy,
                             int coff, hipStream_t stream);
int sd_launch_inception_mean(const bf16_t* x, float* out, int B, int HW, int C, hipStream_t stream);
int sd_launch_inception_resize(const unsigned char* img, void* out, int B, int H, int W, int S, int out_fp32, hipStream_t stream);
```

sonicdiffusionbayeslab_amd/csrc/model.h:

```cpp
#pragma once
#include "../../include/sd_hip.h"
#include "common.h"
#include "kernels.h"

#include <string.h>
#include <sys/mman.h>

#include <algorithm>
#include <map>
#include <new>
#include <set>
#include <string>
#include <tuple>
#include <unordered_map>
#include <vector>

namespace sdhip {

constexpr size_t NOFF = (size_t)-1;
constexpr int T_LATENTS = -2, T_EPS = -3;

struct ParamSpec {
    std::string name;
    std::vector<long long> shape;
    std::vector<float> data;
    bool loaded = false;
    long long numel() const {
        long long n = 1;
        for (auto s : shape) n *= s;
        return n;
    }
};

struct Wrap {
    int type;
    int block_i, layer_i;
};

enum OpKind { OP_SINUSOID, OP_GEMV, OP_CONV_IN, OP_GN, OP_CONV3, OP_GEMM, OP_LN, OP_ATTN, OP_CONV_OUT, OP_SOFTMAX, OP_PQCONV,
              OP_CLIP_EMBED, OP_CLIP_ATTN, OP_QGELU, OP_TO_F32, OP_XATTN, OP_REPLICATE,
              OP_VIT_PREP, OP_VIT_EMBED, OP_VIT_ATTN, OP_POOL, OP_CONV_IN_IMG, OP_ENC_OUT, OP_IP_XATTN };

constexpr int REP_TEXT_POOLED = 2;

struct Op {
    int kind = 0;
    int x1 = -1, x2 = -1, r = -1, out = -1, aux = -1, b2t = -1;
    size_t w = NOFF, b = NOFF, g = NOFF, be = NOFF;
    long b2idx = 0;
    int M = 0, N = 0, K = 0, K1 = 0, epi = 0;
    int B = 0, Hin = 0, Win = 0, Cin = 0, Hout = 0, Wout = 0, stride = 1, up = 0;
    int C1 = 0, C2 = 0, HW = 0, silu = 0, nsplit = 0;
    float eps = 0.f;
    int heads = 0, D = 0, Nq = 0, Nk = 0;
    long ldq = 0, ldk = 0, ldv = 0, ldo = 0, qoff = 0, koff = 0, voff = 0;
    int silu_in = 0, splitk = 1;
    int pool_by_ids = 0;
    int defer = 0, slab_t = -1, slab_k = 0, slab_r = -1, slab_b2t = -1;
    size_t slab_b = NOFF;
    long slab_b2idx = 0;
    int wt = -1;
    size_t wx = NOFF;
    long xoff = 0, woff_el = 0, coff = 0, ldx_o = 0, ldw_o = 0, ldc_o = 0;
    float scale = 0.f;
    long wbs = 0;
    int rpb = 0, sm_valid = 0;
    int dt = 0, out_fp8 = 0, Cpad = 0, Kalg = 0;
    int sname = -1;
    int stats = -1, s1 = -1, s2 = -1;
    int subpix = 0;
    int asym = 0;
    int hm = 0;
    int qps = 0;
    int rs = -1, lnrs = -1, lnnp = 0;
    size_t c1 = NOFF;
    size_t wsc = NOFF;
    float xs = 1.f, os = 1.f;
    int scx1 = -1, scx2 = -1, scc1 = 0, scc2 = 0;
    size_t scw = NOFF;
    int nwrap = 0;
    Wrap wraps[3];
};

struct HostBlob {
    unsigned char* p = nullptr;
    size_t n = 0, cap = 0;
    unsigned char* data() { return p; }
    const unsigned char* data() const { return p; }
    size_t size() const { return n; }
    bool empty() const { return n == 0; }
    bool reserve(size_t bytes) {
        if (bytes <= cap) return true;
        void* q = mmap(nullptr, bytes, PROT_READ | PROT_WRITE, MAP_PRIVATE | MAP_ANONYMOUS | MAP_POPULATE, -1, 0);
        if (q == MAP_FAILED) return false;
        (void)madvise(q, bytes, MADV_HUGEPAGE);
        if (p) { memcpy(q, p, n); munmap(p, cap); }
        p = (unsigned char*)q; cap = bytes;
        return true;
    }
    void resize(size_t bytes) {
        if (bytes > cap && !reserve(std::max(bytes, cap * 2))) throw std::bad_alloc();
        n = bytes;
    }
    void release() { if (p) munmap(p, cap); p = nullptr; n = cap = 0; }
    ~HostBlob() { release(); }
    HostBlob() = default;
    HostBlob(const HostBlob&) = delete;
    HostBlob& operator=(const HostBlob&) = delete;
};

struct Tn {
    size_t bytes = 0;
    int def = -1, last = -1;
    bool persistent = false;
    bool ctx = false;
    bool ctx_ip = false;
    size_t off = NOFF;
};

struct Plan {
    int UB = 0, branch = -1;
    int rep = 1;
    int lh = 0, lw = 0;
    int ip = 0;
    struct IpFold { int at, bt, C; size_t wqT, wo, wkv; };
    std::vector<IpFold> ip_fold;
    int ip_e = -1, ip_proj = -1, ip_tok = -1, ip_kv = -1;
    std::vector<Tn> tensors;
    std::vector<Op> ops;
    std::vector<char> skipped;
    std::vector<int> ctx_kv;
    std::vector<size_t> ctx_w;
    std::vector<int> ctx_c;
    int ctx_bf16 = -1;
    struct Fold { int kv, at, bw, C; size_t wqT, wo; bool perm; int c2 = -1; size_t lnu = NOFF; int c1 = -1; size_t ones = NOFF; };
    std::vector<Fold> ctx_fold;
    int ctx_fold_scratch = -1;
    std::map<std::string, int> taps;
    size_t total_bytes = 0;
    ClipPrepGeom geom;
    std::vector<int> prep_tab;
    const int* dtab = nullptr;
};

}

struct sd_unet {
    int kind = 0;
    sd_unet_config cfg;
    sd_clip_config clip;
    sd_clip_vision_config vis;
    int text_proj = 0;
    int eos_id = -1;
    std::map<std::pair<int, int>, int*> prep_tabs;
    std::vector<sdhip::ParamSpec> params;
    std::unordered_map<std::string, int> pindex;
    std::unordered_map<std::string, size_t> woff;
    sdhip::HostBlob hblob;
    char* dweights = nullptr;
    bool finalized = false;
    bool debug_taps = false;
    bool fp8 = false;
    float s_norm = 8.f, s_ff = 2.f;
    std::vector<std::string> act_names;
    std::unordered_map<std::string, int> act_index;
    std::vector<float> act_scale, act_amax;
    int act_id(const std::string& name, float dflt) {
        auto it = act_index.find(name);
        if (it != act_index.end()) return it->second;
        act_index[name] = (int)act_names.size();
        act_names.push_back(name); act_scale.push_back(dflt); act_amax.push_back(0.f);
        return (int)act_names.size() - 1;
    }
    std::map<std::tuple<int, int, int, int, int, int>, sdhip::Plan> plans;
    int last_rep = 1, last_ip = 0;
    int last_h = 0, last_w = 0;
    std::unordered_map<std::string, long> tproj_off;
    long tproj_total = 0;
    float* dcond = nullptr;
    bool cond_set = false;
    float* dinpaint = nullptr;
    size_t inpaint_cap = 0;
    int inpaint_b = 0, inpaint_h = 0, inpaint_w = 0;
    std::set<std::tuple<int, int, int, int>> ip_keys;
};

namespace sdhip {

void enumerate_params(sd_unet* u);
void enumerate_params_vae(sd_unet* u);
void enumerate_params_vae_encoder(sd_unet* u);
void enumerate_params_clip(sd_unet* u);
void enumerate_params_vit(sd_unet* u);
int pack_all(sd_unet* u);
double pack_alloc_seconds();
inline std::string clip_layer(int i) { return "text_model.encoder.layers." + std::to_string(i) + "."; }
inline std::string vit_layer(int i) { return "vision_model.encoder.layers." + std::to_string(i) + "."; }
inline int vit_kp(const sd_clip_vision_config& c) { return (3 * c.patch_size * c.patch_size + 63) / 64 * 64; }

int plan_rep(const sd_unet* u, int latent_batch, int unet_batch);
int check_latent_size(const sd_unet* u, int lh, int lw, const char* who);
int get_plan(sd_unet* u, int UB, int branch, Plan** out, int rep = 1, int lh = -1, int lw = -1, int ip = 0);
bool ip_active(const sd_unet* u, int UB, int branch, int lh, int lw);

int ensure_zero_page();
const void* zero_page();
int check_image_size(int H, int W, const char* who);
int run_op(sd_unet* u, const Plan& pl, const Op& o, char* ws, const float* latents, int latent_batch, float* eps_out,
           float timestep, hipStream_t stream);

void* op_scratch(size_t bytes);

}
```

sonicdiffusionbayeslab_amd/csrc/ops.hip:

```cpp
#include "model.h"

#include <stdlib.h>

namespace sdhip {

static void* g_scratch = nullptr;
static size_t g_scratch_bytes = 0;
void* op_scratch(size_t bytes) {
    if (bytes > g_scratch_bytes) {
        (void)hipDeviceSynchronize();
        if (g_scratch) (void)hipFree(g_scratch);
        g_scratch = nullptr;
        g_scratch_bytes = 0;
        if (hipMalloc(&g_scratch, bytes) != hipSuccess) return nullptr;
        g_scratch_bytes = bytes;
    }
    return g_scratch;
}

}

using namespace sdhip;

static void conv3x3_args(GemmArgs& a, const void* X, const void* W, const float* bias, const float* bias2, const void* R, void* Y,
// ... 303 lines not shown
    if (hipMalloc((void**)&tmp, (size_t)B * 3 * g.R * S) != hipSuccess) {
        (void)hipFree(dtab);
        SD_REQUIRE(false, "clip_preprocess: cannot allocate the intermediate");
    }
    int rc = 0;
    if (hipMemcpy(dtab, tab.data(), tab.size() * sizeof(int), hipMemcpyHostToDevice) != hipSuccess) {
        sd_set_error("clip_preprocess: tap table upload failed");
        rc = -2;
    }
    if (!rc) rc = sd_launch_clip_preprocess(images, B, g, dtab, tmp, (bf16_t*)patches, P, Kp, crop, (hipStream_t)stream);
    if (!rc && hipStreamSynchronize((hipStream_t)stream) != hipSuccess) {
        sd_set_error("clip_preprocess: stream synchronisation failed");
        rc = -2;
    }
    (void)hipFree(tmp);
    (void)hipFree(dtab);
    return rc;
}

extern "C" int sd_op_gemm_qkv_headmajor(void* stream, const void* X, long long ldx, const void* W, void* Q, void* KV, int M,
                                        int C, int tokens, int K) {
    if (ensure_zero_page()) return -2;
    GemmArgs a;
    a.X = (const bf16_t*)X; a.ldx = ldx; a.K1 = K; a.W = (const bf16_t*)W; a.C = (bf16_t*)Q; a.ldc = C; a.M = M; a.N = 3 * C;
    a.K = K; a.zero_page = zero_page(); a.splitk = 1; a.KV = (bf16_t*)KV; a.hm_C = C; a.hm_tok = tokens;
    return sd_launch_gemm(a, 0, (hipStream_t)stream);
}

extern "C" int sd_op_attention_headmajor(void* stream, const void* Q, long long ldq, const void* K, const void* V, void* O,
                                         long long ldo, int B, int heads, int Nq, int Nk, int D, float scale) {
    AttnArgs a;
    a.Q = (const bf16_t*)Q; a.ldq = ldq; a.K = (const bf16_t*)K; a.V = (const bf16_t*)V; a.kv_head_major = 1;
    a.O = (bf16_t*)O; a.ldo = ldo; a.B = B; a.heads = heads; a.Nq = Nq; a.Nk = Nk; a.D = D; a.scale = scale;
    if (ensure_zero_page()) return -2;
    a.consts = zero_page();
    return sd_launch_attention(a, (hipStream_t)stream);
}

extern "C" int sd_op_conv_in_cond(void* stream, const float* x, int Bsrc, const float* cond, int Bcond, const float* Wt,
                                  const float* bias, void* y, int B, int H, int W, int Cout) {
    return sd_launch_conv_in_cond(x, Bsrc, cond, Bcond, Wt, bias, (bf16_t*)y, B, H, W, Cout, (hipStream_t)stream);
}

extern "C" int sd_op_conv_in(void* stream, const float* x, int Bsrc, const float* Wt, const float* bias, void* y, int B,
                             int H, int W, int Cin, int Cout) {
    return sd_launch_conv_in(x, Bsrc, Wt, bias, (bf16_t*)y, B, H, W, Cin, Cout, (hipStream_t)stream);
}

extern "C" int sd_op_conv_out(void* stream, const void* x, const void* Wp, const float* bias, float* y, int B, int H,
                              int W, int Cin, int Cout) {
    return sd_launch_conv_out((const bf16_t*)x, (const bf16_t*)Wp, bias, y, B, H, W, Cin, Cout, (hipStream_t)stream);
}

extern "C" int sd_op_time_embedding(void* stream, float t, const void* W1, const float* b1, const void* W2,
                                    const float* b2, float* scratch, float* temb, int dim_in, int dim) {
    int rc;
    if ((rc = sd_launch_timestep_sinusoid(t, scratch, dim_in, (hipStream_t)stream))) return rc;
    if ((rc = sd_launch_gemv(scratch, (const bf16_t*)W1, b1, scratch + dim_in, dim, dim_in, 0, (hipStream_t)stream))) return rc;
    return sd_launch_gemv(scratch + dim_in, (const bf16_t*)W2, b2, temb, dim, dim, 1, (hipStream_t)stream);
}

extern "C" int sd_op_timestep_cond(void* stream, float t, const float* cond, const void* Wc, float* row, float* emb,
                                   int cond_dim, int dim) {
    SD_REQUIRE(cond && Wc && row && emb, "timestep_cond: null operand");
    SD_REQUIRE(((uintptr_t)cond & 15) == 0 && cond_dim > 0, "timestep_cond: cond must be 16-byte aligned, cond_dim > 0");
    int rc;
    if ((rc = sd_launch_gemv(cond, (const bf16_t*)Wc, nullptr, row, dim, cond_dim, 0, (hipStream_t)stream))) return rc;
    return sd_launch_timestep_sinusoid_row(t, row, emb, dim, (hipStream_t)stream);
}

extern "C" int sd_op_gemm_fp8(void* stream, const void* X, long long ldx, const void* W, const float* wscale, float xscale,
                              const float* bias, const void* R, long long ldr, void* C, long long ldc, int M, int N, int K,
                              int epi, int out_fp8, float oscale) {
    if (ensure_zero_page()) return -2;
    SD_REQUIRE(epi == 0 || epi == 1, "sd_op_gemm_fp8: epi %d (0 = std, 1 = GEGLU)", epi);
    SD_REQUIRE(xscale > 0.f && (!out_fp8 || (epi == 1 && oscale > 0.f)), "sd_op_gemm_fp8: bad scales / fp8 output needs the GEGLU epilogue");
    GemmArgs a;
    a.X = (const bf16_t*)X; a.ldx = ldx; a.K1 = K; a.W = (const bf16_t*)W; a.bias = bias; a.R = (const bf16_t*)R; a.ldr = ldr;
    a.C = (bf16_t*)C; a.ldc = ldc; a.M = M; a.N = N; a.K = K; a.zero_page = zero_page();
    a.dt = 1; a.wscale = wscale; a.xscale_inv = 1.0f / xscale; a.out_fp8 = out_fp8; a.oscale = oscale;
    a.splitk = epi ? 1 : op_gemm_splitk(M, N, K, 1);
    if (splitk_slab(a, "sd_op_gemm_fp8")) return -1;
    return sd_launch_gemm(a, epi, (hipStream_t)stream);
}

extern "C" int sd_op_conv3x3_fp8(void* stream, const void* X, const void* W, const float* wscale, float xscale,
                                 const float* bias, const float* bias2, const void* R, void* Y, int B, int Hin, int Win,
                                 int Cin, int Cout, int stride, int upsample) {
    if (ensure_zero_page()) return -2;
    SD_REQUIRE(stride == 1 || stride == 2, "conv3x3 fp8: stride %d", stride);
    SD_REQUIRE(xscale > 0.f, "conv3x3 fp8: activation scale");
    GemmArgs a;
    conv3x3_args(a, X, W, bias, bias2, R, Y, B, Hin, Win, Cin, Cout, stride, upsample ? 1 : 0);
    a.dt = 1; a.wscale = wscale; a.xscale_inv = 1.0f / xscale;
    a.splitk = sd_conv3x3_splitk(a.M, a.N, Cin, Hin, Win, stride, a.up, 1);
    if (splitk_slab(a, "sd_op_conv3x3_fp8")) return -1;
    return sd_launch_conv3x3(a, (hipStream_t)stream);
}

extern "C" int sd_op_groupnorm_fp8(void* stream, const void* x1, int C1, const void* x2, int C2, const float* gamma,
                                   const float* beta, void* y, int B, int HW, int groups, float eps, int silu, int Cpad,
                                   float oscale) {
    GroupNormArgs a;
    a.x1 = (const bf16_t*)x1; a.C1 = C1; a.x2 = (const bf16_t*)x2; a.C2 = C2; a.gamma = gamma; a.beta = beta;
    a.y = (bf16_t*)y; a.B = B; a.HW = HW; a.groups = groups; a.eps = eps; a.silu = silu;
    a.out_fp8 = 1; a.Cpad = Cpad; a.oscale = oscale;
    a.nsplit = sd_groupnorm_nsplit(B, HW);
    a.partial = (float*)op_scratch(sd_groupnorm_scratch_bytes(B, HW, groups));
    SD_REQUIRE(a.partial, "sd_op_groupnorm_fp8: cannot allocate scratch");
    return sd_launch_groupnorm(a, (hipStream_t)stream);
}

extern "C" int sd_op_layernorm_fp8(void* stream, const void* x, const float* gamma, const float* beta, void* y, int rows,
                                   int C, int Cpad, float eps, float oscale) {
    return sd_launch_layernorm_fp8((const bf16_t*)x, gamma, beta, y, rows, C, Cpad, eps, oscale, (hipStream_t)stream);
}

extern "C" int sd_op_quantize_fp8(void* stream, const void* x_bf16, void* y_fp8, long long rows, int C, int Cpad, float scale) {
    return sd_launch_quantize_fp8((const bf16_t*)x_bf16, y_fp8, (long)rows, C, Cpad, scale, (hipStream_t)stream);
}

extern "C" int sd_op_amax_e4m3(void* stream, const void* codes, long long nbytes, unsigned* out_code) {
    SD_REQUIRE(out_code, "sd_op_amax_e4m3: null output");
    SD_CHECK_HIP(hipMemsetAsync(out_code, 0, sizeof(unsigned), (hipStream_t)stream));
    return sd_launch_amax_e4m3(codes, (long)nbytes, out_code, (hipStream_t)stream);
}

extern "C" int sd_op_ln_partials(int kind, int M, int N) { return kind == 0 ? (N + 159) / 160 * 2 : 2 * sd_xattn_slices(M, N); }
extern "C" int sd_op_gemm_rowstats(void* stream, const void* X, long long ldx, const void* W, const float* bias, const void* R,
                                   long long ldr, void* C, long long ldc, int M, int N, int K, float* rowstats) {
    if (ensure_zero_page()) return -2;
    SD_REQUIRE(rowstats, "sd_op_gemm_rowstats: null partials buffer");
    GemmArgs a;
    a.X = (const bf16_t*)X; a.ldx = ldx; a.K1 = K; a.W = (const bf16_t*)W; a.bias = bias; a.R = (const bf16_t*)R; a.ldr = ldr;
    a.C = (bf16_t*)C; a.ldc = ldc; a.M = M; a.N = N; a.K = K; a.zero_page = zero_page(); a.splitk = 1; a.rowstats = rowstats;
    return sd_launch_gemm(a, 0, (hipStream_t)stream);
}
extern "C" int sd_op_gemm_plan(void* stream, const void* X, long long ldx, const void* X2, long long ldx2, int K1, const void* W,
                               const float* bias, const float* bias2, const void* R, long long ldr, void* C, long long ldc,
                               int M, int N, int K, float* rowstats, float* stats, const float* ln_rs, int ln_parts,
                               const float* ln_c1, float ln_eps, void* KV, int hm_tokens) {
    if (ensure_zero_page()) return -2;
    GemmArgs a;
    a.X = (const bf16_t*)X; a.ldx = ldx; a.X2 = (const bf16_t*)X2; a.ldx2 = ldx2; a.K1 = K1; a.W = (const bf16_t*)W;
    a.bias = bias; a.bias2 = bias2; a.R = (const bf16_t*)R; a.ldr = ldr; a.C = (bf16_t*)C; a.ldc = ldc; a.M = M; a.N = N; a.K = K;
    a.zero_page = zero_page(); a.splitk = 1; a.rowstats = rowstats; a.stats = stats;
    a.ln_rs = ln_rs; a.ln_np = ln_parts; a.ln_c1 = ln_c1; a.ln_eps = ln_eps;
    if (hm_tokens > 0) {
        SD_REQUIRE(N % 3 == 0 && KV, "sd_op_gemm_plan: head-major K / V needs N = 3 C and a KV buffer");
        a.KV = (bf16_t*)KV; a.hm_C = N / 3; a.hm_tok = hm_tokens;
    }
    return sd_launch_gemm(a, 0, (hipStream_t)stream);
}
extern "C" int sd_op_gemm_ln(void* stream, const void* X, long long ldx, const void* Wg, const float* c1, const float* c2,
                             const float* rowstats, int parts, float eps, void* C, long long ldc, int M, int N, int K, int epi) {
    if (ensure_zero_page()) return -2;
    SD_REQUIRE(epi == 0 || epi == 1, "sd_op_gemm_ln: epi %d (0 = plain, 1 = GEGLU)", epi);
    GemmArgs a;
    a.X = (const bf16_t*)X; a.ldx = ldx; a.K1 = K; a.W = (const bf16_t*)Wg; a.bias = c2;
    a.C = (bf16_t*)C; a.ldc = ldc; a.M = M; a.N = N; a.K = K; a.zero_page = zero_page(); a.splitk = 1;
    a.ln_rs = rowstats; a.ln_np = parts; a.ln_c1 = c1; a.ln_eps = eps;
    return sd_launch_gemm(a, epi, (hipStream_t)stream);
}

extern "C" int sd_op_xattn_fused_rowstats(void* stream, const void* X, const void* R, void* Y, const void* At, const void* Bw,
                                          const float* bias, int M, int C, int rows_per_sample, int L, float* rowstats) {
    SD_REQUIRE(sd_xattn_fused_applicable(rows_per_sample, C, 8, L), "sd_op_xattn_fused_rowstats: shape not supported");
    XattnArgs a = xattn_args(X, R, Y, At, Bw, bias, M, C, rows_per_sample, L);
    a.rowstats = rowstats;
    return sd_launch_xattn_fused(a, (hipStream_t)stream);
}

extern "C" int sd_op_ip_xattn(void* stream, const void* R, void* Rout, const void* A, const void* Bt, const float* gamma,
                              const float* beta, float eps, long long M, int C, int rows_per_sample, int heads, int T) {
    return sd_launch_ip_xattn((const bf16_t*)R, (bf16_t*)Rout, (const bf16_t*)A, (const bf16_t*)Bt, gamma, beta, eps, (long)M, C,
                              rows_per_sample, heads, T, (hipStream_t)stream);
}

extern "C" int sd_op_xattn_fused(void* stream, const void* X, const void* R, void* Y, const void* At, const void* Bw,
                                 const float* bias, int M, int C, int rows_per_sample, int L) {
    SD_REQUIRE(sd_xattn_fused_applicable(rows_per_sample, C, 8, L) || getenv("SD_XATTN_FUSED"),
               "sd_op_xattn_fused: shape not supported (8 heads x 80 key slots, 64 < L <= 80, C %% 32 == 0, tokens per sample %% 128 == 0)");
    return sd_launch_xattn_fused(xattn_args(X, R, Y, At, Bw, bias, M, C, rows_per_sample, L), (hipStream_t)stream);
}

extern "C" int sd_op_xattn_fused_ln(void* stream, const void* X, const void* R, void* Y, const void* At, const void* Bw,
                                    const float* bias, int M, int C, int rows_per_sample, int L, const float* ln_rowstats,
                                    int ln_parts, long long ln_rows, const float* c2, float eps, float* rowstats) {
    SD_REQUIRE(sd_xattn_fused_applicable(rows_per_sample, C, 8, L), "sd_op_xattn_fused_ln: shape not supported");
    SD_REQUIRE(ln_rowstats && c2, "sd_op_xattn_fused_ln: null operand");
    XattnArgs a = xattn_args(X, R, Y, At, Bw, bias, M, C, rows_per_sample, L);
    a.rowstats = rowstats;
    a.ln_rs = ln_rowstats; a.ln_np = ln_parts; a.ln_rows = ln_rows; a.ln_c2 = c2; a.ln_eps = eps;
    return sd_launch_xattn_fused(a, (hipStream_t)stream);
}

extern "C" int sd_op_xattn_fused_stamps(void* stream, const void* X, const void* R, void* Y, const void* At, const void* Bw,
                                        const float* bias, int M, int C, int rows_per_sample, int L, unsigned long long* stamps) {
    SD_REQUIRE(stamps, "sd_op_xattn_fused_stamps: null stamp buffer");
    SD_REQUIRE(sd_xattn_fused_applicable(rows_per_sample, C, 8, L), "sd_op_xattn_fused_stamps: shape not supported");
    XattnArgs a = xattn_args(X, R, Y, At, Bw, bias, M, C, rows_per_sample, L);
    a.stamps = stamps;
    return sd_launch_xattn_fused(a, (hipStream_t)stream);
}
```

sonicdiffusionbayeslab_amd/csrc/plan.hip:

```cpp
#include "model.h"

#include <stdlib.h>

namespace sdhip {

namespace {

struct Builder {
    sd_unet* u;
    Plan& pl;
    int UB;
    std::vector<Wrap> wrapstack;
    std::map<int, int> stats_of;
    std::map<int, float> tscale;
    static std::string stem(const std::string& key) {
        const size_t n = key.rfind(".weight");
        return n == std::string::npos ? key : key.substr(0, n);
    }
    std::string error;
    float xscale(int t) {
        auto it = tscale.find(t);
        if (it == tscale.end()) {
            if (error.empty()) error = "fp8 consumer of a tensor without a scale";
            return 1.0f;
        }
        return it->second;
    }
    bool producer_stats = !(getenv("SD_GN_PRODUCER_STATS") && atoi(getenv("SD_GN_PRODUCER_STATS")) == 0);
    void want_stats(Op& o, int M, int N) {
        if (!producer_stats || u->kind != 0 || o.splitk > 1 || M % 64 != 0 || o.epi != 0 || o.rpb != 0) return;
        o.stats = tensor((size_t)(M / 64) * N * 2 * 4);
        stats_of[o.out] = o.stats;
    }

    int prefix_rep = 1;
    int replicate(int t, size_t bytes, int r) {
        Op o; o.kind = OP_REPLICATE; o.x1 = t; o.M = (int)(bytes / 16); o.N = r; o.out = tensor(bytes * r);
        push(o);
        return o.out;
    }
    bool ln_fold = !(getenv("SD_LN_FOLD") && atoi(getenv("SD_LN_FOLD")) == 0);
    int want_rowstats(Op& o, int M, int C, int& rs) {
        int np = 0;
        if (o.kind == OP_GEMM && o.epi == 0 && o.splitk == 1 && !o.out_fp8 && o.N == C && o.M == M && o.ldc_o == 0) np = (C + 159) / 160 * 2;
        else if (o.kind == OP_XATTN && o.N == C && o.M == M) np = 2 * sd_xattn_slices(M, C);
        static const bool big_tiles = getenv("SD_GEMM_BIG") != nullptr;
        if (!ln_fold || np == 0 || np > 16 || C < 128 || big_tiles) return 0;
        o.rs = rs = tensor((size_t)np * M * 2 * 4);
        return np;
    }
    int gemm_ln(int x, int rs, int np, int M, int N, int C, const std::string& w, int epi) {
        Op o; o.kind = OP_GEMM; o.x1 = x; o.K1 = o.K = o.Kalg = C; o.M = M; o.N = N; o.epi = epi; o.splitk = 1;
        o.w = W(w + ".ln"); o.c1 = W(w + ".c1"); o.b = W(w + ".c2"); o.lnrs = rs; o.lnnp = np;
        o.out = tensor((size_t)M * (epi ? N / 2 : N) * 2);
        push(o);
        return o.out;
    }

    int ctx_tensor(size_t bytes) {
        const int id = tensor(bytes, true);
        pl.tensors[id].ctx = true;
        return id;
    }
    int ctx_ip_tensor(size_t bytes) {
        const int id = ctx_tensor(bytes);
        pl.tensors[id].ctx_ip = true;
        return id;
    }
    int tensor(size_t bytes, bool persistent = false) {
        Tn t;
        t.bytes = (bytes + 255) / 256 * 256;
        t.persistent = persistent;
        pl.tensors.push_back(t);
        return (int)pl.tensors.size() - 1;
    }
    size_t W(const std::string& k) {
        auto it = u->woff.find(k);
        if (it == u->woff.end()) {
            if (error.empty()) error = "missing packed weight " + k;
            return 0;
        }
        return it->second;
    }
    Op& push(Op op) {
        op.nwrap = (int)wrapstack.size();
        for (int i = 0; i < op.nwrap; ++i) op.wraps[i] = wrapstack[i];
        pl.ops.push_back(op);
        return pl.ops.back();
    }
    static int pad128(int c) { return (c + 127) / 128 * 128; }
    int gn(int x1, int c1, int x2, int c2, int hw, const std::string& g, const std::string& b, float eps, int silu,
           bool fq = false) {
        Op o; o.kind = OP_GN; o.x1 = x1; o.C1 = c1; o.x2 = x2; o.C2 = c2; o.HW = hw; o.B = UB;
        o.g = W(g); o.be = W(b); o.eps = eps; o.silu = silu;
        o.nsplit = sd_groupnorm_nsplit(UB, hw);
        o.aux = tensor(sd_groupnorm_scratch_bytes(UB, hw, u->cfg.norm_num_groups));
        if (hw % 64 == 0 && !sd_groupnorm_uses_small(UB, hw, c1, c2, u->cfg.norm_num_groups) && stats_of.count(x1) &&
            (x2 < 0 || stats_of.count(x2))) {
            o.s1 = stats_of[x1];
            o.s2 = x2 >= 0 ? stats_of[x2] : -1;
        }
        if (fq) {
            o.out_fp8 = 1; o.Cpad = pad128(c1 + c2); o.sname = u->act_id(stem(g), u->s_norm); o.os = u->act_scale[o.sname];
            o.out = tensor((size_t)UB * hw * o.Cpad); tscale[o.out] = o.os;
        } else o.out = tensor((size_t)UB * hw * (c1 + c2) * 2);
        push(o);
        return o.out;
    }
    int conv3(int x, int hin, int win, int cin, int cout, int stride, int up, const std::string& w, const std::string& b,
              long b2idx, int b2t, int r, bool fq = false) {
        Op o; o.kind = OP_CONV3; o.x1 = x; o.B = UB; o.Hin = hin; o.Win = win; o.Cin = cin; o.N = cout;
        o.stride = stride; o.up = up;
        o.Hout = ((hin << up) + 2 - 3) / stride + 1;
        o.Wout = ((win << up) + 2 - 3) / stride + 1;
        o.M = UB * o.Hout * o.Wout; o.K = 9 * cin; o.Kalg = o.K;
        o.b = W(b); o.b2t = b2t; o.b2idx = b2idx; o.r = r;
        if (fq) { o.dt = 1; o.Cin = pad128(cin); o.K = 9 * o.Cin; o.w = W(w + ".fp8"); o.wsc = W(w + ".scale"); o.xs = xscale(x); }
        else o.w = W(w);
        static const bool subpix_off = getenv("SD_CONV_SUBPIXEL") && atoi(getenv("SD_CONV_SUBPIXEL")) == 0;
        if (up && !fq && !subpix_off && u->kind == 0 && stride == 1 && r < 0 && b2t < 0 && (hin * win) % 64 == 0 &&
            u->woff.count(w + ".sub")) {
            o.subpix = 1; o.K = 4 * cin; o.Kalg = 4 * cin;
            o.w = W(w + ".sub"); o.splitk = 1;
            o.out = tensor((size_t)o.M * cout * 2);
            if ((hin * win) % 128 == 0) want_stats(o, o.M, cout);
            push(o);
            return o.out;
        }
        o.splitk = sd_conv3x3_splitk(o.M, o.N, o.Cin, hin, win, stride, up, o.dt);
        if (o.splitk > 1) o.aux = tensor((size_t)o.splitk * o.M * o.N * 4);
        o.out = tensor((size_t)o.M * cout * 2);
        GemmArgs g;
        g.M = o.M; g.N = o.N; g.Cin = o.Cin; g.K = o.K; g.ldw = o.K; g.Hin = hin; g.Win = win; g.Hout = o.Hout; g.Wout = o.Wout;
        g.stride = stride; g.up = up; g.dt = o.dt;
        if (sd_conv_halo_mode(g) != 2) want_stats(o, o.M, cout);
        push(o);
        return o.out;
    }
    int gemm(int x1, int k1, int x2, int k2, int M, int N, const std::string& w, const std::string& b, int r, int epi,
             bool fq = false, const std::string& oname = "") {
        Op o; o.kind = OP_GEMM; o.x1 = x1; o.x2 = x2; o.K1 = k1; o.K = k1 + k2; o.Kalg = o.K; o.M = M; o.N = N; o.epi = epi;
        o.b = b.empty() ? NOFF : W(b); o.r = r;
        if (fq) { o.dt = 1; o.K = o.K1 = pad128(k1); o.w = W(w + ".fp8"); o.wsc = W(w + ".scale"); o.xs = xscale(x1); }
        else o.w = W(w);
        o.splitk = epi ? 1 : sd_gemm_splitk(M, N, o.dt ? o.K / 2 : o.K, o.dt ? 128 : 0);
        if (o.splitk > 1) o.aux = tensor((size_t)o.splitk * M * N * 4);
        if (!oname.empty()) {
            o.out_fp8 = 1; o.sname = u->act_id(oname, u->s_ff); o.os = u->act_scale[o.sname]; o.Cpad = pad128(N / 2);
            o.out = tensor((size_t)M * o.Cpad); tscale[o.out] = o.os;
        } else o.out = tensor((size_t)M * (epi ? N / 2 : N) * 2);
        push(o);
        return o.out;
    }
    int ln(int x, int M, int C, const std::string& g, const std::string& b, bool fq = false) {
        Op o; o.kind = OP_LN; o.x1 = x; o.M = M; o.N = C; o.g = W(g); o.be = W(b); o.eps = 1e-5f;
        if (fq) {
            o.out_fp8 = 1; o.Cpad = pad128(C); o.sname = u->act_id(stem(g), u->s_norm); o.os = u->act_scale[o.sname];
            o.out = tensor((size_t)M * o.Cpad); tscale[o.out] = o.os;
        } else o.out = tensor((size_t)M * C * 2);
        push(o);
        return o.out;
    }
    int attn(int q, long qoff, long ldq, int kv, long koff, long voff, long ldkv, int nq, int nk, int C) {
        Op o; o.kind = OP_ATTN; o.x1 = q; o.x2 = kv; o.qoff = qoff; o.koff = koff; o.voff = voff;
        o.ldq = ldq; o.ldk = o.ldv = ldkv; o.ldo = C; o.B = UB; o.heads = u->cfg.num_heads; o.D = C / u->cfg.num_heads;
        o.Nq = nq; o.Nk = nk;
        o.out = tensor((size_t)UB * nq * C * 2);
        push(o);
        return o.out;
    }
    bool shortcut_fuse = !(getenv("SD_SHORTCUT_FUSE") && atoi(getenv("SD_SHORTCUT_FUSE")) == 0);
    int resnet(const std::string& p, int x1, int c1, int x2, int c2, int cout, int rh, int rw, int tproj_t) {
        const int hw = rh * rw, cin = c1 + c2, M = UB * hw;
        const bool fq = u->fp8;
        int t1 = gn(x1, c1, x2, c2, hw, p + "norm1.weight", p + "norm1.bias", u->cfg.norm_eps, 1, fq);
        int t2 = conv3(t1, rh, rw, cin, cout, 1, 0, p + "conv1.weight", p + "conv1.bias", u->tproj_off.at(p), tproj_t, -1, fq);
        int t3 = gn(t2, cout, -1, 0, hw, p + "norm2.weight", p + "norm2.bias", u->cfg.norm_eps, 1, fq);
        int sc = x1;
        if (cin != cout) {
            GemmArgs g;
            g.M = M; g.N = cout; g.Cin = cout; g.K = 9 * cout; g.ldw = g.K; g.Hin = g.Hout = rh; g.Win = g.Wout = rw;
            g.Csc1 = c1; g.Csc2 = x2 >= 0 ? c2 : 0;
            if (shortcut_fuse && !fq && u->kind == 0 && u->woff.count(p + "conv2.bias+shortcut") && sd_conv_halo_shortcut_applicable(g)) {
                const int out = conv3(t3, rh, rw, cout, cout, 1, 0, p + "conv2.weight", p + "conv2.bias+shortcut", 0, -1, -1, fq);
                Op& o = pl.ops.back();
                o.scx1 = x1; o.scc1 = c1; o.scx2 = x2; o.scc2 = g.Csc2; o.scw = W(p + "conv_shortcut.weight");
                o.Kalg += cin;
                return out;
            }
            sc = gemm(x1, c1, x2, c2, M, cout, p + "conv_shortcut.weight", p + "conv_shortcut.bias", -1, 0);
        }
        return conv3(t3, rh, rw, cout, cout, 1, 0, p + "conv2.weight", p + "conv2.bias", 0, -1, sc, fq);
    }
    int n_transformers = 0;
    int transformer(const std::string& p, int x, int C, int rh, int rw) {
        const int hw = rh * rw, L = u->cfg.context_len;
        int M = UB * hw;
        const std::string t = p + "transformer_blocks.0.";
        const bool fq = u->fp8;
        int g = gn(x, C, -1, 0, hw, p + "norm.weight", p + "norm.bias", 1e-6f, 0, fq);
        int h0 = gemm(g, C, -1, 0, M, C, p + "proj_in.weight", p + "proj_in.bias", -1, 0, fq);
        int qkv, rs = -1, np = 0;
        if (!fq && (np = want_rowstats(pl.ops.back(), M, C, rs)) > 0) {
            qkv = gemm_ln(h0, rs, np, M, 3 * C, C, t + "attn1.qkv.weight", 0);
        } else {
            int n1 = ln(h0, M, C, t + "norm1.weight", t + "norm1.bias", fq);
            qkv = gemm(n1, C, -1, 0, M, 3 * C, t + "attn1.qkv.weight", "", -1, 0, fq);
        }
        static const bool hm_off = (getenv("SD_ATTN_HEADMAJOR") && atoi(getenv("SD_ATTN_HEADMAJOR")) == 0) ||
                                   getenv("SD_ATTN_NO_PIPE") || getenv("SD_ATTN_NO_DMA") || getenv("SD_GEMM_BIG");
        const bool hm = !hm_off && C / u->cfg.num_heads == 40 && C % 160 == 0 && hw % 128 == 0 && hw >= 256 &&
                        sd_gemm_tile_rows(M, 3 * C) == 128 && pl.ops.back().splitk == 1;
        int a1;
        if (hm) {
            pl.ops.back().hm = 1;
            pl.ops.back().HW = hw;
            a1 = attn(qkv, 0, C, qkv, (long)M * C, 2l * M * C, C, hw, hw, C);
            pl.ops.back().hm = 1;
        } else {
            a1 = attn(qkv, 0, 3 * C, qkv, C, 2 * C, 3 * C, hw, hw, C);
        }
        pl.ops.back().qps = 1;
        int h1 = gemm(a1, C, -1, 0, M, C, t + "attn1.to_out.0.weight", t + "attn1.to_out.0.bias", h0, 0);
        const int to_out_op = (int)pl.ops.size() - 1;
        if (prefix_rep > 1) {
            x = replicate(x, (size_t)M * C * 2, prefix_rep);
            h1 = replicate(h1, (size_t)M * C * 2, prefix_rep);
            UB *= prefix_rep;
            M = UB * hw;
            prefix_rep = 1;
        }
        static const int fused_min_hw = getenv("SD_XATTN_FUSED") ? atoi(getenv("SD_XATTN_FUSED")) : 1024;
        static const int fold_max_hw = getenv("SD_XATTN_FOLD") ? atoi(getenv("SD_XATTN_FOLD")) : 1024;
        static const bool xln_off = getenv("SD_XATTN_LN") && atoi(getenv("SD_XATTN_LN")) == 0;
        const int NH = u->cfg.num_heads, NP = NH * 80;
        const int xmode = (fused_min_hw > 0 && hw >= fused_min_hw && sd_xattn_fused_applicable(hw, C, NH, L)) ? 0
                          : (hw <= fold_max_hw && hw % 128 == 0 && L <= 80) ? 1 : 2;
        int rs2 = -1, np2 = 0;
        const long rs2_rows = (long)pl.ops[to_out_op].M;
        const bool first_tf = n_transformers++ == 0;
        if (!fq && !xln_off && (xmode == 0 || (!first_tf && rs2_rows == M)) &&
            u->woff.count(t + (xmode == 2 ? "attn2.to_q.weight.ln" : "attn2.to_q.weight.T.ln"))) {
            if (first_tf) pl.ops[to_out_op].splitk = 1;
            np2 = want_rowstats(pl.ops[to_out_op], (int)rs2_rows, C, rs2);
        }
        int n2 = np2 > 0 ? h1 : ln(h1, M, C, t + "norm2.weight", t + "norm2.bias");
        int kv = ctx_tensor((size_t)UB * L * 2 * C * 2);
        pl.ctx_kv.push_back(kv);
        pl.ctx_w.push_back(W(t + "attn2.kv.weight"));
        pl.ctx_c.push_back(C);
        int res = h1;
        if (pl.ip) {
            const int at = ctx_ip_tensor((size_t)UB * 32 * C * 2), bt = ctx_ip_tensor((size_t)UB * C * 32 * 2);
            pl.ip_fold.push_back(Plan::IpFold{at, bt, C, W(t + "attn2.to_q.weight.T"), W(t + "attn2.to_out.0.weight"), W(t + "attn2.kv_ip.weight")});
            Op o; o.kind = OP_IP_XATTN; o.x1 = h1; o.wt = at; o.x2 = bt; o.M = M; o.N = C; o.rpb = hw; o.heads = NH;
            o.g = W(t + "norm2.weight"); o.be = W(t + "norm2.bias"); o.eps = 1e-5f;
            o.out = tensor((size_t)M * C * 2); push(o); res = o.out;
        }
        int h2;
        if (xmode == 0) {
            int at = ctx_tensor((size_t)UB * NP * C * 2), bw = ctx_tensor((size_t)UB * C * NP * 2);
            Plan::Fold fd{kv, at, bw, C, W(t + (np2 > 0 ? "attn2.to_q.weight.T.ln" : "attn2.to_q.weight.T")), W(t + "attn2.to_out.0.weight"), true};
            if (np2 > 0) { fd.c2 = ctx_tensor((size_t)UB * NP * 4); fd.lnu = W(t + "attn2.to_q.lnu"); }
            pl.ctx_fold.push_back(fd);
            Op o; o.kind = OP_XATTN; o.x1 = n2; o.r = res; o.wt = at; o.x2 = bw; o.M = M; o.N = C; o.K = NP; o.rpb = hw;
            o.sm_valid = L; o.b = W(t + "attn2.to_out.0.bias"); o.heads = NH;
            if (np2 > 0) { o.lnrs = rs2; o.lnnp = np2; o.s1 = fd.c2; o.ldx_o = rs2_rows; }
            o.out = tensor((size_t)M * C * 2); push(o); h2 = o.out;
        } else if (xmode == 1) {
            int at = ctx_tensor((size_t)UB * NP * C * 2), bw = ctx_tensor((size_t)UB * C * NP * 2);
            Plan::Fold fd{kv, at, bw, C, W(t + (np2 > 0 ? "attn2.to_q.weight.T.ln" : "attn2.to_q.weight.T")), W(t + "attn2.to_out.0.weight"), false};
            if (np2 > 0) {
                fd.c2 = ctx_tensor((size_t)UB * NP * 4); fd.lnu = W(t + "attn2.to_q.lnu");
                fd.c1 = ctx_tensor((size_t)UB * NP * 4); fd.ones = W(t + "attn2.to_q.ones");
            }
            pl.ctx_fold.push_back(fd);
            int pr;
            { Op o; o.kind = OP_GEMM; o.x1 = n2; o.K1 = C; o.K = C; o.M = M; o.N = NP; o.epi = 2; o.sm_valid = L;
              o.wt = at; o.wbs = (long)NP * C; o.rpb = hw;
              if (np2 > 0) { o.lnrs = rs2; o.lnnp = np2; o.s1 = fd.c1; o.s2 = fd.c2; }
              o.out = tensor((size_t)M * NP * 2); push(o); pr = o.out; }
            { Op o; o.kind = OP_GEMM; o.x1 = pr; o.K1 = NP; o.K = NP; o.M = M; o.N = C; o.epi = 0;
              o.wt = bw; o.wbs = (long)C * NP; o.rpb = hw; o.b = W(t + "attn2.to_out.0.bias"); o.r = res;
              o.out = tensor((size_t)M * C * 2); push(o); h2 = o.out; }
        } else {
            int q2 = np2 > 0 ? gemm_ln(h1, rs2, np2, M, C, C, t + "attn2.to_q.weight", 0)
                             : gemm(n2, C, -1, 0, M, C, t + "attn2.to_q.weight", "", -1, 0);
            int a2 = attn(q2, 0, C, kv, 0, C, 2 * C, hw, L, C);
            h2 = gemm(a2, C, -1, 0, M, C, t + "attn2.to_out.0.weight", t + "attn2.to_out.0.bias", res, 0);
        }
        int ff;
        if (!fq && (np = want_rowstats(pl.ops.back(), M, C, rs)) > 0) {
            ff = gemm_ln(h2, rs, np, M, 8 * C, C, t + "ff.geglu.weight", 1);
        } else {
            int n3 = ln(h2, M, C, t + "norm3.weight", t + "norm3.bias", fq);
            ff = gemm(n3, C, -1, 0, M, 8 * C, t + "ff.geglu.weight", t + "ff.geglu.bias", -1, 1, fq, fq ? t + "ff.net.0" : std::string());
        }
        static const bool merge_off = getenv("SD_FF_MERGE") && atoi(getenv("SD_FF_MERGE")) == 0;
        int out;
        if (!fq && !merge_off) {
            out = gemm(ff, 4 * C, h2, C, M, C, p + "ff_out.weight", p + "ff_out.bias", x, 0);
        } else {
            int h3 = gemm(ff, 4 * C, -1, 0, M, C, t + "ff.net.2.weight", t + "ff.net.2.bias", h2, 0, fq);
            out = gemm(h3, C, -1, 0, M, C, p + "proj_out.weight", p + "proj_out.bias", x, 0);
        }
        if (pl.ops.back().splitk == 1 && sd_gemm_tile_rows(M, C, pl.ops.back().K) == 128) want_stats(pl.ops.back(), M, C);
        return out;
    }

    int vae_resnet(const std::string& p, int x, int cin, int cout, int rh, int rw) {
        const int hw = rh * rw, M = UB * hw;
        int t1 = gn(x, cin, -1, 0, hw, p + "norm1.weight", p + "norm1.bias", 1e-6f, 1);
        int t2 = conv3(t1, rh, rw, cin, cout, 1, 0, p + "conv1.weight", p + "conv1.bias", 0, -1, -1);
        int t3 = gn(t2, cout, -1, 0, hw, p + "norm2.weight", p + "norm2.bias", 1e-6f, 1);
        int sc = x;
        if (cin != cout) sc = gemm(x, cin, -1, 0, M, cout, p + "conv_shortcut.weight", p + "conv_shortcut.bias", -1, 0);
        return conv3(t3, rh, rw, cout, cout, 1, 0, p + "conv2.weight", p + "conv2.bias", 0, -1, sc);
    }
    int vae_attention(const std::string& p, int x, int C, int rh, int rw) {
        const int hw = rh * rw, M = UB * hw;
        const int qc = hw <= 4096 ? hw : 2048;
        int g = gn(x, C, -1, 0, hw, p + "group_norm.weight", p + "group_norm.bias", 1e-6f, 0);
        int qk = gemm(g, C, -1, 0, M, 2 * C, p + "qk.weight", p + "qk.bias", -1, 0);
        const int vT = tensor((size_t)UB * C * hw * 2), S = tensor((size_t)qc * hw * 2), O = tensor((size_t)M * C * 2);
        for (int img = 0; img < UB; ++img) {
            {
                Op o; o.kind = OP_GEMM; o.wx = W(p + "to_v.weight"); o.ldx_o = C; o.K1 = C; o.K = C; o.M = C; o.N = hw;
                o.wt = g; o.woff_el = (long)img * hw * C; o.ldw_o = C;
                o.out = vT; o.coff = (long)img * C * hw; o.ldc_o = hw;
                push(o);
            }
            for (int q0 = 0; q0 < hw; q0 += qc) {
                const int rows = std::min(qc, hw - q0);
                {
                    Op o; o.kind = OP_GEMM; o.x1 = qk; o.xoff = ((long)img * hw + q0) * 2 * C; o.ldx_o = 2 * C; o.K1 = C; o.K = C;
                    o.M = rows; o.N = hw; o.wt = qk; o.woff_el = (long)img * hw * 2 * C + C; o.ldw_o = 2 * C;
                    o.out = S; o.ldc_o = hw;
                    push(o);
                }
                { Op o; o.kind = OP_SOFTMAX; o.x1 = S; o.out = S; o.M = rows; o.N = hw; o.scale = 1.0f / sqrtf((float)C); push(o); }
                {
                    Op o; o.kind = OP_GEMM; o.x1 = S; o.ldx_o = hw; o.K1 = hw; o.K = hw; o.M = rows; o.N = C;
                    o.wt = vT; o.woff_el = (long)img * C * hw; o.ldw_o = hw; o.b = W(p + "to_v.bias");
                    o.out = O; o.coff = ((long)img * hw + q0) * C; o.ldc_o = C;
                    push(o);
                }
            }
        }
        return gemm(O, C, -1, 0, M, C, p + "to_out.0.weight", p + "to_out.0.bias", x, 0);
    }
    void build_vae() {
        const sd_unet_config& c = u->cfg;
        const int nl = c.num_levels, top = c.block_out_channels[nl - 1];
        int rh = pl.lh, rw = pl.lw;
        int t_pq = tensor((size_t)UB * c.in_channels * rh * rw * 4);
        { Op o; o.kind = OP_PQCONV; o.x1 = T_LATENTS; o.out = t_pq; o.B = UB; o.HW = rh * rw;
          o.w = W("post_quant_conv.weight"); o.b = W("post_quant_conv.bias"); push(o); }
        int h;
        { Op o; o.kind = OP_CONV_IN; o.x1 = t_pq; o.B = UB; o.Hin = rh; o.Win = rw; o.Cin = c.in_channels; o.N = top;
          o.w = W("decoder.conv_in.weight"); o.b = W("decoder.conv_in.bias"); o.out = tensor((size_t)UB * rh * rw * top * 2);
          push(o); h = o.out; }
        pl.taps["conv_in"] = h;
        h = vae_resnet("decoder.mid_block.resnets.0.", h, top, top, rh, rw);
        h = vae_attention("decoder.mid_block.attentions.0.", h, top, rh, rw);
        h = vae_resnet("decoder.mid_block.resnets.1.", h, top, top, rh, rw);
        pl.taps["mid"] = h;
        int ch = top;
        for (int i = 0; i < nl; ++i) {
            const int co = c.block_out_channels[nl - 1 - i];
            const std::string bp = "decoder.up_blocks." + std::to_string(i) + ".";
            for (int j = 0; j < c.layers_per_block + 1; ++j) {
                h = vae_resnet(bp + "resnets." + std::to_string(j) + ".", h, ch, co, rh, rw);
                ch = co;
            }
            if (i < nl - 1) {
                h = conv3(h, rh, rw, co, co, 1, 1, bp + "upsamplers.0.conv.weight", bp + "upsamplers.0.conv.bias", 0, -1, -1);
                rh *= 2; rw *= 2;
            }
            pl.taps["up" + std::to_string(i)] = h;
        }
        int g = gn(h, ch, -1, 0, rh * rw, "decoder.conv_norm_out.weight", "decoder.conv_norm_out.bias", 1e-6f, 1);
        { Op o; o.kind = OP_CONV_OUT; o.x1 = g; o.out = T_EPS; o.B = UB; o.Hin = rh; o.Win = rw; o.Cin = ch; o.N = c.out_channels;
          o.w = W("decoder.conv_out.weight"); o.b = W("decoder.conv_out.bias"); push(o); }
    }

    void build_vae_encoder() {
        const sd_unet_config& c = u->cfg;
        const int nl = c.num_levels, top = c.block_out_channels[nl - 1], c0 = c.block_out_channels[0];
        int rh = pl.lh << (nl - 1), rw = pl.lw << (nl - 1);
        int h;
        { Op o; o.kind = OP_CONV_IN_IMG; o.x1 = T_LATENTS; o.B = UB; o.Hin = rh; o.Win = rw; o.Cin = c.out_channels; o.N = c0;
          o.w = W("encoder.conv_in.weight"); o.b = W("encoder.conv_in.bias"); o.out = tensor((size_t)UB * rh * rw * c0 * 2);
          push(o); h = o.out; }
        pl.taps["conv_in"] = h;
        int ch = c0;
        for (int i = 0; i < nl; ++i) {
            const int co = c.block_out_channels[i];
            const std::string bp = "encoder.down_blocks." + std::to_string(i) + ".";
            for (int j = 0; j < c.layers_per_block; ++j) {
                h = vae_resnet(bp + "resnets." + std::to_string(j) + ".", h, ch, co, rh, rw);
                ch = co;
            }
            if (i < nl - 1) {
                h = conv3(h, rh, rw, co, co, 2, 0, bp + "downsamplers.0.conv.weight", bp + "downsamplers.0.conv.bias", 0, -1, -1);
                pl.ops.back().asym = 1;
                rh /= 2; rw /= 2;
            }
            pl.taps["down" + std::to_string(i)] = h;
        }
        h = vae_resnet("encoder.mid_block.resnets.0.", h, top, top, rh, rw);
        h = vae_attention("encoder.mid_block.attentions.0.", h, top, rh, rw);
        h = vae_resnet("encoder.mid_block.resnets.1.", h, top, top, rh, rw);
        pl.taps["mid"] = h;
        int g = gn(h, top, -1, 0, rh * rw, "encoder.conv_norm_out.weight", "encoder.conv_norm_out.bias", 1e-6f, 1);
        { Op o; o.kind = OP_ENC_OUT; o.x1 = g; o.out = T_EPS; o.B = UB; o.Hin = rh; o.Win = rw; o.Cin = top; o.N = 2 * c.in_channels;
          o.w = W("encoder.conv_out.weight"); o.b = W("encoder.conv_out.bias");
          o.g = W("quant_conv.weight"); o.be = W("quant_conv.bias"); push(o); }
    }

    int clip_encoder_layer(const std::string& p, int t, int M, int L, int H, int I, int heads, int attn_kind, bool gelu = false) {
        const std::string a = p + "self_attn.";
        int n1 = ln(t, M, H, p + "layer_norm1.weight", p + "layer_norm1.bias");
        int qkv = gemm(n1, H, -1, 0, M, 3 * H, a + "qkv.weight", a + "qkv.bias", -1, 0);
        int at;
        if (attn_kind == OP_VIT_ATTN && H / heads == 80) {
            Op o; o.kind = OP_ATTN; o.x1 = qkv; o.x2 = qkv; o.qoff = 0; o.koff = H; o.voff = 2 * H; o.ldq = o.ldk = o.ldv = 3 * H;
            o.ldo = H; o.B = UB; o.heads = heads; o.D = 80; o.Nq = L; o.Nk = L;
            o.out = tensor((size_t)M * H * 2); push(o); at = o.out;
        } else {
            Op o; o.kind = attn_kind; o.x1 = qkv; o.B = UB; o.Nq = L; o.N = H; o.heads = heads;
            o.out = tensor((size_t)M * H * 2); push(o); at = o.out;
        }
        t = gemm(at, H, -1, 0, M, H, a + "out_proj.weight", a + "out_proj.bias", t, 0);
        int n2 = ln(t, M, H, p + "layer_norm2.weight", p + "layer_norm2.bias");
        int f = gemm(n2, H, -1, 0, M, I, p + "mlp.fc1.weight", p + "mlp.fc1.bias", -1, 0);
        { Op o; o.kind = OP_QGELU; o.x1 = f; o.out = f; o.M = M; o.N = I; o.epi = gelu ? 1 : 0; push(o); }
        return gemm(f, I, -1, 0, M, H, p + "mlp.fc2.weight", p + "mlp.fc2.bias", t, 0);
    }

    void build_clip() {
        const sd_clip_config& c = u->clip;
        const int L = c.max_positions, H = c.hidden_size, I = c.intermediate_size, M = UB * L;
        int t;
        { Op o; o.kind = OP_CLIP_EMBED; o.x1 = T_LATENTS; o.M = M; o.N = H; o.Nk = L;
          o.w = W("text_model.embeddings.token_embedding.weight"); o.g = W("text_model.embeddings.position_embedding.weight");
          o.out = tensor((size_t)M * H * 2); push(o); t = o.out; }
        for (int i = 0; i < c.num_layers; ++i) {
            t = clip_encoder_layer(clip_layer(i), t, M, L, H, I, c.num_heads, OP_CLIP_ATTN);
            pl.taps["layer" + std::to_string(i)] = t;
        }
        if (pl.rep == REP_TEXT_POOLED) {
            int pr;
            { Op o; o.kind = OP_POOL; o.x1 = t; o.pool_by_ids = 1; o.B = UB; o.Nq = L; o.N = H; o.out = tensor((size_t)UB * H * 2); push(o); pr = o.out; }
            int f = ln(pr, UB, H, "text_model.final_layer_norm.weight", "text_model.final_layer_norm.bias");
// ... 309 lines not shown
```

sonicdiffusionbayeslab_amd/csrc/unet.hip:

```cpp
#include "model.h"

#include <stdarg.h>
#include <stdio.h>
#include <stdlib.h>

#include <chrono>

static thread_local char g_err[1024] = "";
void sd_set_error(const char* fmt, ...) {
    va_list ap;
    va_start(ap, fmt);
    vsnprintf(g_err, sizeof(g_err), fmt, ap);
    va_end(ap);
}
extern "C" const char* sd_last_error(void) { return g_err; }
extern "C" int sd_abi_version(void) { return 3; }

static void* g_zero_page = nullptr;

namespace sdhip {

int ensure_zero_page() {
    if (g_zero_page) return 0;
    SD_CHECK_HIP(hipMalloc(&g_zero_page, 4096));
    SD_CHECK_HIP(hipMemset(g_zero_page, 0, 4096));
    const unsigned short one_chunk[8] = {0x3F80, 0, 0, 0, 0, 0, 0, 0};
    SD_CHECK_HIP(hipMemcpy((char*)g_zero_page + 256, one_chunk, sizeof(one_chunk), hipMemcpyHostToDevice));
    return 0;
}
const void* zero_page() { return g_zero_page; }

int run_op(sd_unet* u, const Plan& pl, const Op& o, char* ws, const float* latents, int latent_batch, float* eps_out,
           float timestep, hipStream_t stream) {
    auto T = [&](int id) -> char* { return id >= 0 ? ws + pl.tensors[id].off : nullptr; };
    const char* wb = u->dweights;
    switch (o.kind) {
        case OP_SINUSOID:
            if (u->cond_set) return sd_launch_timestep_sinusoid_row(timestep, u->dcond, (float*)T(o.out), o.N, stream);
            return sd_launch_timestep_sinusoid(timestep, (float*)T(o.out), o.N, stream);
        case OP_GEMV:
            return sd_launch_gemv((const float*)T(o.x1), (const bf16_t*)(wb + o.w), (const float*)(wb + o.b),
                                  (float*)T(o.out), o.N, o.K, o.silu_in, stream);
        case OP_CONV_IN:
            if (u->kind == 0 && o.Cin == 9) {
                SD_REQUIRE(u->inpaint_b > 0, "forward: this UNet has in_channels = 9 and no inpainting condition is set "
                                             "(sd_unet_set_inpaint_cond_hw: mask and masked-image latents)");
                SD_REQUIRE(u->inpaint_h == o.Hin && u->inpaint_w == o.Win && o.B % u->inpaint_b == 0,
                           "forward: the inpainting condition was set for batch %d at %dx%d, the forward runs batch %d at %dx%d",
                           u->inpaint_b, u->inpaint_h, u->inpaint_w, o.B, o.Hin, o.Win);
                return sd_launch_conv_in_cond(latents, latent_batch, u->dinpaint, u->inpaint_b, (const float*)(wb + o.w),
                                              (const float*)(wb + o.b), (bf16_t*)T(o.out), o.B, o.Hin, o.Win, o.N, stream);
            }
            return sd_launch_conv_in(o.x1 >= 0 ? (const float*)T(o.x1) : latents, o.x1 >= 0 ? o.B : latent_batch,
                                     (const float*)(wb + o.w), (const float*)(wb + o.b), (bf16_t*)T(o.out), o.B, o.Hin,
                                     o.Win, o.Cin, o.N, stream);
        case OP_PQCONV:
            return sd_launch_pqconv(latents, (const float*)(wb + o.w), (const float*)(wb + o.b), (float*)T(o.out), o.B,
                                    o.HW, timestep , stream);
        case OP_SOFTMAX:
            if (o.N > 4096) return sd_launch_softmax_rows_long((bf16_t*)T(o.x1), o.M, o.N, o.scale, stream);
            return sd_launch_softmax_rows((bf16_t*)T(o.x1), o.M, o.N, o.scale, stream);
        case OP_GN: {
            GroupNormArgs a;
            a.x1 = (const bf16_t*)T(o.x1); a.C1 = o.C1; a.x2 = (const bf16_t*)T(o.x2); a.C2 = o.C2;
            a.gamma = (const float*)(wb + o.g); a.beta = (const float*)(wb + o.be);
            a.y = (bf16_t*)T(o.out); a.partial = (float*)T(o.aux);
            a.B = o.B; a.HW = o.HW; a.groups = u->cfg.norm_num_groups; a.nsplit = o.nsplit; a.eps = o.eps; a.silu = o.silu;
            a.out_fp8 = o.out_fp8; a.Cpad = o.Cpad; a.oscale = o.os;
            a.stats1 = (const float*)T(o.s1); a.stats2 = (const float*)T(o.s2);
            if (o.slab_t >= 0) {
                a.slab = (const float*)T(o.slab_t); a.splitk = o.slab_k; a.x1w = (bf16_t*)T(o.x1);
                a.sbias = o.slab_b != NOFF ? (const float*)(wb + o.slab_b) : nullptr;
                a.sbias2 = o.slab_b2t >= 0 ? (const float*)T(o.slab_b2t) + o.slab_b2idx : nullptr;
                a.sR = (const bf16_t*)T(o.slab_r); a.sldr = o.C1;
            }
            return sd_launch_groupnorm(a, stream);
        }
        case OP_CONV3: {
            GemmArgs a;
            a.X = (const bf16_t*)T(o.x1); a.W = (const bf16_t*)(wb + o.w); a.bias = (const float*)(wb + o.b);
            a.bias2 = o.b2t >= 0 ? (const float*)T(o.b2t) + o.b2idx : nullptr;
            a.R = (const bf16_t*)T(o.r); a.ldr = o.N; a.C = (bf16_t*)T(o.out); a.ldc = o.N;
            a.M = o.M; a.N = o.N; a.K = o.K; a.K1 = o.K;
            a.Hin = o.Hin; a.Win = o.Win; a.Cin = o.Cin; a.Hout = o.Hout; a.Wout = o.Wout; a.stride = o.stride; a.up = o.up;
            a.zero_page = g_zero_page; a.splitk = o.splitk; a.slab = (float*)T(o.aux); a.defer_reduce = o.defer;
            if (o.dt) { a.dt = 1; a.wscale = (const float*)(wb + o.wsc); a.xscale_inv = 1.0f / o.xs; }
            a.stats = (float*)T(o.stats);
            a.asym = o.asym;
            if (o.subpix) { a.subpix = 1; a.up = 0; a.w_batch_stride = (long)o.N * 4 * o.Cin; }
            if (o.scw != NOFF) {
                a.Xs1 = (const bf16_t*)T(o.scx1); a.Csc1 = o.scc1; a.Xs2 = (const bf16_t*)T(o.scx2); a.Csc2 = o.scc2;
                a.Wsc = (const bf16_t*)(wb + o.scw); a.ldwsc = o.scc1 + o.scc2;
            }
            return sd_launch_conv3x3(a, stream);
        }
        case OP_GEMM: {
            GemmArgs a;
            a.X = o.wx != NOFF ? (const bf16_t*)(wb + o.wx) : (const bf16_t*)T(o.x1) + o.xoff;
            a.ldx = o.ldx_o ? o.ldx_o : o.K1; a.X2 = (const bf16_t*)T(o.x2); a.ldx2 = o.K - o.K1; a.K1 = o.K1;
            a.W = o.wt >= 0 ? (const bf16_t*)T(o.wt) + o.woff_el : (const bf16_t*)(wb + o.w); a.ldw = o.ldw_o;
            a.bias = o.b != NOFF ? (const float*)(wb + o.b) : nullptr;
            a.R = (const bf16_t*)T(o.r); a.ldr = o.N; a.C = (bf16_t*)T(o.out) + o.coff;
            a.ldc = o.ldc_o ? o.ldc_o : (o.epi == 1 ? o.N / 2 : o.N);
            a.M = o.M; a.N = o.N; a.K = o.K; a.zero_page = g_zero_page; a.splitk = o.splitk; a.slab = (float*)T(o.aux);
            a.defer_reduce = o.defer;
            a.w_batch_stride = o.wbs; a.rows_per_batch = o.rpb; a.sm_valid = o.sm_valid;
            if (o.dt) { a.dt = 1; a.wscale = (const float*)(wb + o.wsc); a.xscale_inv = 1.0f / o.xs; }
            if (o.out_fp8) { a.out_fp8 = 1; a.oscale = o.os; a.ldc = o.Cpad; }
            a.stats = (float*)T(o.stats);
            a.rowstats = (float*)T(o.rs);
            if (o.hm) { a.hm_C = o.N / 3; a.hm_tok = o.HW; a.ldc = a.hm_C; a.KV = (bf16_t*)T(o.out) + (long)o.M * a.hm_C; }
            if (o.lnrs >= 0) { a.ln_rs = (const float*)T(o.lnrs); a.ln_np = o.lnnp; a.ln_c1 = (const float*)(wb + o.c1); a.ln_eps = 1e-5f; }
            if (o.lnrs >= 0 && o.s1 >= 0) { a.ln_c1 = (const float*)T(o.s1); a.bias = (const float*)T(o.s2); a.ln_per_sample = 1; }
            return sd_launch_gemm(a, o.epi, stream);
        }
        case OP_LN:
            if (o.out_fp8)
                return sd_launch_layernorm_fp8((const bf16_t*)T(o.x1), (const float*)(wb + o.g), (const float*)(wb + o.be),
                                               T(o.out), o.M, o.N, o.Cpad, o.eps, o.os, stream);
            return sd_launch_layernorm((const bf16_t*)T(o.x1), (const float*)(wb + o.g), (const float*)(wb + o.be),
                                       (bf16_t*)T(o.out), o.M, o.N, o.eps, stream);
        case OP_ATTN: {
            AttnArgs a;
            a.Q = (const bf16_t*)T(o.x1) + o.qoff; a.ldq = o.ldq;
            a.K = (const bf16_t*)T(o.x2) + o.koff; a.ldk = o.ldk;
            a.V = (const bf16_t*)T(o.x2) + o.voff; a.ldv = o.ldv;
            a.O = (bf16_t*)T(o.out); a.ldo = o.ldo;
            a.B = o.B; a.heads = o.heads; a.Nq = o.Nq; a.Nk = o.Nk; a.D = o.D;
            a.scale = 1.0f / sqrtf((float)o.D);
            a.q_prescaled = o.qps;
            a.consts = g_zero_page;
            a.kv_head_major = o.hm;
            return sd_launch_attention(a, stream);
        }
        case OP_XATTN: {
            XattnArgs a;
            a.X = (const bf16_t*)T(o.x1); a.R = (const bf16_t*)T(o.r); a.Y = (bf16_t*)T(o.out);
            a.At = (const bf16_t*)T(o.wt); a.Bw = (const bf16_t*)T(o.x2); a.bias = (const float*)(wb + o.b);
            a.M = o.M; a.C = o.N; a.rows_per_sample = o.rpb; a.L = o.sm_valid;
            a.rowstats = (float*)T(o.rs);
            if (o.lnrs >= 0) {
                a.ln_rs = (const float*)T(o.lnrs); a.ln_np = o.lnnp; a.ln_rows = o.ldx_o; a.ln_c2 = (const float*)T(o.s1); a.ln_eps = 1e-5f;
            }
            return sd_launch_xattn_fused(a, stream);
        }
        case OP_IP_XATTN:
            return sd_launch_ip_xattn((const bf16_t*)T(o.x1), (bf16_t*)T(o.out), (const bf16_t*)T(o.wt), (const bf16_t*)T(o.x2),
                                      (const float*)(wb + o.g), (const float*)(wb + o.be), o.eps, o.M, o.N, o.rpb, o.heads,
                                      u->cfg.ip_adapter_tokens, stream);
        case OP_REPLICATE:
            return sd_launch_replicate(T(o.x1), T(o.out), (long)o.M * 16, o.N, stream);
        case OP_CLIP_EMBED:
            return sd_launch_clip_embed((const int*)latents, (const bf16_t*)(wb + o.w), (const bf16_t*)(wb + o.g),
                                        (bf16_t*)T(o.out), o.M, o.Nk, o.N, u->clip.vocab_size, stream);
        case OP_CLIP_ATTN:
            return sd_launch_clip_attention((const bf16_t*)T(o.x1), (bf16_t*)T(o.out), o.B, o.Nq, o.N, o.heads, stream);
        case OP_QGELU:
            if (o.epi) return sd_launch_gelu_erf((bf16_t*)T(o.x1), (long)o.M * o.N, stream);
            return sd_launch_quick_gelu((bf16_t*)T(o.x1), (long)o.M * o.N, stream);
        case OP_VIT_PREP:
            return sd_launch_clip_preprocess((const unsigned char*)latents, o.B, pl.geom, pl.dtab, (unsigned char*)T(o.aux),
                                             (bf16_t*)T(o.out), o.Cin, o.K, nullptr, stream);
        case OP_VIT_EMBED:
            return sd_launch_vit_embed((const bf16_t*)T(o.x1), (const float*)(wb + o.b), (const bf16_t*)(wb + o.g),
                                       (bf16_t*)T(o.out), o.B, o.Nq, o.N, stream);
        case OP_VIT_ATTN:
            return sd_launch_vit_attention((const bf16_t*)T(o.x1), (bf16_t*)T(o.out), o.B, o.Nq, o.N, o.heads, stream);
        case OP_POOL:
            return sd_launch_pool_rows((const bf16_t*)T(o.x1), o.pool_by_ids ? (const int*)latents : nullptr, o.B, o.Nq, o.N, u->eos_id,
                                       (bf16_t*)T(o.out), stream);
        case OP_TO_F32:
            return sd_launch_bf16_to_f32((const bf16_t*)T(o.x1), eps_out, (long)o.M * o.N, stream);
        case OP_CONV_IN_IMG:
            return sd_launch_conv_in_image(latents, (const float*)(wb + o.w), (const float*)(wb + o.b), (bf16_t*)T(o.out), o.B,
                                           o.Hin, o.Win, o.N, stream);
        case OP_ENC_OUT:
            return sd_launch_vae_enc_out((const bf16_t*)T(o.x1), (const bf16_t*)(wb + o.w), (const float*)(wb + o.b),
                                         (const float*)(wb + o.g), (const float*)(wb + o.be), eps_out, o.B, o.Hin, o.Win, o.Cin,
                                         stream);
        case OP_CONV_OUT:
            return sd_launch_conv_out((const bf16_t*)T(o.x1), (const bf16_t*)(wb + o.w), (const float*)(wb + o.b), eps_out,
                                      o.B, o.Hin, o.Win, o.Cin, o.N, stream);
    }
    sd_set_error("unet: unknown op kind %d", o.kind);
    return -1;
}

}

using namespace sdhip;

static sd_unet* new_handle(int kind, const sd_unet_config* cfg) {
    sd_unet* u = new sd_unet();
    u->kind = kind;
    if (cfg) {
        u->cfg = *cfg;
        if (kind != 0) u->cfg.time_cond_proj_dim = u->cfg.ip_adapter_tokens = u->cfg.ip_adapter_embed_dim = 0;
        u->debug_taps = getenv("SD_DEBUG_TAPS") != nullptr;
    } else {
        memset(&u->cfg, 0, sizeof(u->cfg));
        u->cfg.num_levels = 1;
    }
    return u;
}

static int check_vae_levels(const sd_unet_config* cfg, const char* who) {
    for (int i = 0; i < cfg->num_levels; ++i) {
        const int c = cfg->block_out_channels[i], cpg = cfg->norm_num_groups ? c / cfg->norm_num_groups : 0;
        SD_REQUIRE(c % 64 == 0 && c % cfg->norm_num_groups == 0 && (cpg >= 8 || cpg == 4),
                   "%s: block_out_channels[%d]=%d must be a multiple of 64 with 4 or >= 8 channels per group", who, i, c);
    }
    return 0;
}

static int check_workspace(const Plan& pl, const char* who, const void* workspace, long long workspace_bytes) {
    SD_REQUIRE((long long)pl.total_bytes <= workspace_bytes, "%s: workspace too small (%lld < %zu)", who, workspace_bytes,
               pl.total_bytes);
    SD_REQUIRE(((uintptr_t)workspace & 255) == 0, "%s: workspace must be 256-byte aligned", who);
    return 0;
}

static int run_plan(sd_unet* u, const Plan& pl, const char* who, void* workspace, long long workspace_bytes, const void* in,
                    int batch, float* out, float scalar, void* stream, int cache_mode = SD_CACHE_OFF) {
    if (check_workspace(pl, who, workspace, workspace_bytes)) return -1;
    for (size_t i = 0; i < pl.ops.size(); ++i) {
        if (cache_mode == SD_CACHE_SKIP && pl.skipped[i]) continue;
        if (int rc = run_op(u, pl, pl.ops[i], (char*)workspace, (const float*)in, batch, out, scalar, (hipStream_t)stream)) return rc;
    }
    return 0;
}

extern "C" int sd_unet_create(const sd_unet_config* cfg, sd_unet** out) {
    SD_REQUIRE(cfg && out, "sd_unet_create: null argument");
    SD_REQUIRE(cfg->num_levels >= 1 && cfg->num_levels <= 8, "sd_unet_create: num_levels %d", cfg->num_levels);
    SD_REQUIRE(cfg->in_channels == 4 || cfg->in_channels == 9,
               "sd_unet_create: in_channels %d (4, or 9 for an inpainting UNet: latents | mask | masked-image latents)",
               cfg->in_channels);
    SD_REQUIRE(cfg->out_channels >= 1 && cfg->out_channels <= 4, "sd_unet_create: out_channels %d", cfg->out_channels);
    for (int i = 0; i < cfg->num_levels; ++i) {
        const int c = cfg->block_out_channels[i];
        SD_REQUIRE(c % 64 == 0 && c % cfg->norm_num_groups == 0 && c / cfg->norm_num_groups >= 8,
                   "sd_unet_create: block_out_channels[%d]=%d must be a multiple of 64 with >= 8 channels per group", i, c);
        if (cfg->attn_levels[i]) {
            const int d = c / cfg->num_heads;
            SD_REQUIRE(c % cfg->num_heads == 0 && (d == 40 || d == 80 || d == 160),
                       "sd_unet_create: head dim %d at level %d not built (40/80/160)", d, i);
        }
    }
    const int dmid = cfg->block_out_channels[cfg->num_levels - 1] / cfg->num_heads;
    SD_REQUIRE(dmid == 40 || dmid == 80 || dmid == 160, "sd_unet_create: mid-block head dim %d not built", dmid);
    SD_REQUIRE(cfg->cross_attention_dim % 64 == 0, "sd_unet_create: cross_attention_dim must be a multiple of 64");
    SD_REQUIRE(cfg->sample_size % (1 << (cfg->num_levels - 1)) == 0, "sd_unet_create: sample_size not divisible");
    SD_REQUIRE(cfg->context_len >= 1, "sd_unet_create: context_len");
    SD_REQUIRE(cfg->weight_dtype == SD_DTYPE_BF16 || cfg->weight_dtype == SD_DTYPE_FP8_E4M3,
               "sd_unet_create: weight_dtype %d (0 = bf16, 1 = fp8 e4m3)", cfg->weight_dtype);
    SD_REQUIRE(cfg->fp8_act_scale_norm >= 0.f && cfg->fp8_act_scale_ff >= 0.f, "sd_unet_create: negative fp8 activation scale");
    SD_REQUIRE(cfg->time_cond_proj_dim >= 0 && cfg->time_cond_proj_dim % 8 == 0,
               "sd_unet_create: time_cond_proj_dim %d must be 0 (none) or a positive multiple of 8 (the GEMV reads 8 at a time)",
               cfg->time_cond_proj_dim);
    if (cfg->ip_adapter_tokens != 0 || cfg->ip_adapter_embed_dim != 0) {
        SD_REQUIRE(cfg->ip_adapter_tokens == 4, "sd_unet_create: ip_adapter_tokens %d (4 image tokens are built: the plain ip-adapter_sd15 "
                   "family; the \"plus\" / \"full-face\" adapters with 16 or 257 tokens are not)", cfg->ip_adapter_tokens);
        SD_REQUIRE(cfg->ip_adapter_embed_dim > 0 && cfg->ip_adapter_embed_dim % 64 == 0,
                   "sd_unet_create: ip_adapter_embed_dim %d must be a positive multiple of 64", cfg->ip_adapter_embed_dim);
        SD_REQUIRE(cfg->cross_attention_dim <= 1536, "sd_unet_create: an IP-Adapter needs cross_attention_dim <= 1536 (the token LayerNorm)");
        for (int i = 0; i < cfg->num_levels; ++i)
// ... 770 lines not shown
```

Measured before the change: 11.30 images/s.

## Route merged FF-out GEMM through conv-halo kernel's wide GEMM-only mode

Adds a GEMM-only mode (SC==2) to the conv halo kernel. It skips the halo geometry and streams X and W tiles through a three-stage LDS pipeline using buffer loads directly to LDS. A new wide launcher, split-K heuristic and applicability check are added. The plan routes the merged ff_out+proj_out GEMM to this path by default, but only when its split-K choice matches the existing heuristic's and is greater than 1. The aim is better load/compute overlap for this large-K GEMM, at the cost of more kernel complexity and new wait-count logic.

```diff
diff --git a/include/sd_hip.h b/include/sd_hip.h
--- a/include/sd_hip.h
+++ b/include/sd_hip.h
@@ -241,6 +241,16 @@
                     const float* bias, const float* bias2, const void* R, long long ldr, void* C, long long ldc, int M, int N,
                     int K, float* rowstats, float* stats, const float* ln_rs, int ln_parts, const float* ln_c1, float ln_eps,
                     void* KV, int hm_tokens);
+int sd_op_gemm_wide(void* stream, const void* X, long long ldx, const void* X2, long long ldx2, int K1, const void* W,
+                    const float* bias, const float* bias2, const void* R, long long ldr, void* C, long long ldc, int M, int N,
+                    int K, float* stats);
+int sd_op_gemm_wide_splitk(int M, int N, int K);
+int sd_op_gemm_wide_applicable(int M, int N, int K, int K1, long long ldx, long long ldx2, long long ldw, long long ldr,
+                               long long ldc, int epi, int features);
+int sd_op_gemm_wide_groupnorm(void* stream, const void* X, long long ldx, const void* X2, long long ldx2, int K1, const void* W,
+                              const float* bias, const float* bias2, const void* R, void* C, int M, int N, int K,
+                              const float* gamma, const float* beta, void* Yn, int B, int groups, float eps, int silu,
+                              int deferred);
 int sd_op_xattn_fused_rowstats(void* stream, const void* X, const void* R, void* Y, const void* At, const void* Bw,
                                const float* bias, int M, int C, int rows_per_sample, int L, float* rowstats);
 int sd_op_ip_xattn(void* stream, const void* R, void* Rout, const void* A, const void* Bt, const float* gamma, const float* beta,
diff --git a/sonicdiffusionbayeslab_amd/_lib.py b/sonicdiffusionbayeslab_amd/_lib.py
--- a/sonicdiffusionbayeslab_amd/_lib.py
+++ b/sonicdiffusionbayeslab_amd/_lib.py
@@ -155,6 +155,11 @@
     "sd_op_gemm_rowstats": (_i, [_vp, _vp, _ll, _vp, _vp, _vp, _ll, _vp, _ll, _i, _i, _i, _vp]),
     "sd_op_gemm_plan": (_i, [_vp, _vp, _ll, _vp, _ll, _i, _vp, _vp, _vp, _vp, _ll, _vp, _ll, _i, _i, _i, _vp, _vp, _vp, _i, _vp, _f,
                             _vp, _i]),
+    "sd_op_gemm_wide": (_i, [_vp, _vp, _ll, _vp, _ll, _i, _vp, _vp, _vp, _vp, _ll, _vp, _ll, _i, _i, _i, _vp]),
+    "sd_op_gemm_wide_splitk": (_i, [_i, _i, _i]),
+    "sd_op_gemm_wide_applicable": (_i, [_i, _i, _i, _i, _ll, _ll, _ll, _ll, _ll, _i, _i]),
+    "sd_op_gemm_wide_groupnorm": (_i, [_vp, _vp, _ll, _vp, _ll, _i, _vp, _vp, _vp, _vp, _vp, _i, _i, _i, _vp, _vp, _vp, _i, _i, _f,
+                                       _i, _i]),
     "sd_op_gemm_ln": (_i, [_vp, _vp, _ll, _vp, _vp, _vp, _vp, _i, _f, _vp, _ll, _i, _i, _i, _i]),
     "sd_op_xattn_fused_rowstats": (_i, [_vp, _vp, _vp, _vp, _vp, _vp, _vp, _i, _i, _i, _i, _vp]),
     "sd_op_xattn_fused": (_i, [_vp, _vp, _vp, _vp, _vp, _vp, _vp, _i, _i, _i, _i]),
diff --git a/sonicdiffusionbayeslab_amd/csrc/conv_halo.hip b/sonicdiffusionbayeslab_amd/csrc/conv_halo.hip
--- a/sonicdiffusionbayeslab_amd/csrc/conv_halo.hip
+++ b/sonicdiffusionbayeslab_amd/csrc/conv_halo.hip
@@ -29,6 +29,11 @@
 __global__ __launch_bounds__(NWV * 64, NWV == 8 ? 2 : 1) void conv_halo_kernel(const GemmArgs p) {
     static_assert(NWV == 8 || (NWV == 4 && DT == 0), "4-wave layout: bf16 only");
     static_assert(!SC || (DT == 0 && DIAG == 0 && NWV == 8 && SUB == 0), "shortcut phase: bf16, 8 waves, 9 taps");
+    static_assert(SC <= 2 && (SC < 2 || GEN == 0), "GEMM-only mode: no geometry");
+    constexpr bool GM = SC == 2;
+    constexpr int NST = 3;
+    constexpr int XSTAGE = BM * 128;
+    static_assert(3 * XSTAGE <= 2 * HBYTES, "three X stages fit the halo buffers");
     static_assert(!SUB || (DT == 0 && DIAG == 0 && NWV == 8), "sub-pixel upsampler: bf16, 8 waves");
     static_assert(!GEN || (SUB == 0 && DIAG == 0 && NWV == 8), "geometry mode: 9 taps, 8 waves");
     constexpr int NTAP = SUB ? 4 : 9;
@@ -56,7 +61,7 @@
     const int Mrows = SUB ? p.M >> 2 : p.M;
 
     const int up = SUB ? 0 : p.up;
-    const int Ho = SUB ? p.Hin : p.Hout, Wo = SUB ? p.Win : p.Wout, HWo = Ho * Wo;
+    const int Ho = GM ? 1 : SUB ? p.Hin : p.Hout, Wo = GM ? 1 : SUB ? p.Win : p.Wout, HWo = Ho * Wo;
     const int RW = GEN ? p.rows_per_batch : min(Ho, BM / Wo);
     const int PW = p.Win + 2, PP = ((RW >> up) + 2) * PW;
     const int PIX = RW * Wo;
@@ -73,7 +78,7 @@
     int hyv[GEN ? HPIECES : 1];
     const int jdup = wave < 2 ? HPIECES - 1 : HPIECES - 2;
 #pragma unroll
-    for (int j = 0; j < HPIECES; ++j) {
+    for (int j = 0; !GM && j < HPIECES; ++j) {
         const int L = (j == HPIECES - 1 ? jdup : j) * NT + tid;
         const int slot = L >> 3, cpos = L & 7;
         const int i = slot / PP, rem = slot - i * PP;
@@ -118,6 +123,7 @@
         }
         m0 = tile_m * BM;
         n0 = tile_n * BN;
+        if (GM) return;
         if (GEN) {
             const int b = tile_m / tpi, y0 = (tile_m - b * tpi) * RW;
             m0 = b * HWo + y0 * Wo;
@@ -187,7 +193,7 @@
     const int lrow = lane & 15, lq = lane >> 4;
     int hbase[TM], hrc[TM];
 #pragma unroll
-    for (int f = 0; f < TM; ++f) {
+    for (int f = 0; !GM && f < TM; ++f) {
         if (GEN) {
             const int pt = min(wm * WTM + f * 16 + lrow, PIX - 1);
             const int row = pt / Wo;
@@ -204,7 +210,8 @@
     const int wswz0 = DT ? ((2 * lq) ^ swz_of(lane, 1)) << 4 : (lq ^ (lane & 7)) << 4;
 
     const int sc_gch = ((lane & 7) ^ (lane >> 3)) << 4;
-    const int scp1 = SC ? p.Csc1 * 2 : 0, scp2 = SC ? p.Csc2 * 2 : 0, scpw = SC ? (int)p.ldwsc * 2 : 0;
+    const int scp1 = GM ? (int)p.ldx * 2 : SC ? p.Csc1 * 2 : 0, scp2 = GM ? (int)p.ldx2 * 2 : SC ? p.Csc2 * 2 : 0;
+    const int scpw = SC ? (int)p.ldwsc * 2 : 0;
     const int vXs1 = (lane >> 3) * scp1 + sc_gch, vXs2 = (lane >> 3) * scp2 + sc_gch, vWs = (lane >> 3) * scpw + sc_gch;
     const int scfrag = (wm * WTM + lrow) * 128 + ((lq ^ (lane & 7)) << 4);
 
@@ -222,7 +229,7 @@
     bf16x8 xf0[TM], wf0[TN], xf1[TM], wf1[TN];
     int xan[TM];
 #pragma unroll
-    for (int f = 0; f < TM; ++f) xan[f] = frag_addr(f, 0);
+    for (int f = 0; !GM && f < TM; ++f) xan[f] = frag_addr(f, 0);
     auto mfmas = [&](const bf16x8* xf, const bf16x8* wf) {
 #pragma unroll
         for (int a = 0; a < TN; ++a)
@@ -239,14 +246,50 @@
     char* const Hb1 = smem + HBYTES;
     char* const Wb = smem + 2 * HBYTES;
 
+    const int gm_kt = GM ? (p.Csc1 + p.Csc2) >> 6 : 0, gm_kt1 = GM ? p.Csc1 >> 6 : 0;
+    auto stage_gm = [&](int t, int st) {
+        char* const xb = smem + st * XSTAGE;
+        char* const wb = Wb + st * WBYTES;
+        const int nsc1 = gm_kt1;
+        const unsigned rows = (unsigned)p.M;
+        const bool seg1 = t < nsc1;
+        const int pitch = seg1 ? scp1 : scp2;
+        const __amdgpu_buffer_rsrc_t rx = __builtin_amdgcn_make_buffer_rsrc((void*)(seg1 ? p.Xs1 : p.Xs2), 0,
+                                                                            (int)(rows * (unsigned)pitch), 0x00020000);
+        const int vx = seg1 ? vXs1 : vXs2;
+        const int so = (m0 + wave * 8) * pitch + (seg1 ? t : t - nsc1) * 128;
+#pragma unroll
+        for (int i = 0; i < BM / 64; ++i)
+            __builtin_amdgcn_raw_ptr_buffer_load_lds(rx, LDS_PTR(xb + (wave + 8 * i) * 1024), 16, vx, so + i * 64 * pitch, 0, 0);
+        const __amdgpu_buffer_rsrc_t rw = __builtin_amdgcn_make_buffer_rsrc((void*)p.Wsc, 0, (int)((unsigned)p.N * (unsigned)scpw), 0x00020000);
+#pragma unroll
+        for (int i = 0; i < WPW; ++i) {
+            const int pc = wpiece(i);
+            __builtin_amdgcn_raw_ptr_buffer_load_lds(rw, LDS_PTR(wb + pc * 1024), 16, vWs, (n0 + pc * 8) * scpw + t * 128, 0, 0);
+        }
+    };
+    int gt_begin = 0, gt_end = 0, gst = 0;
+    auto gm_prologue = [&]() {
+        gt_begin = (int)((long)gm_kt * split / p.splitk);
+        gt_end = (int)((long)gm_kt * (split + 1) / p.splitk);
+        stage_gm(gt_begin, gst);
+        if (gt_begin + 1 < gt_end) stage_gm(gt_begin + 1, gst == NST - 1 ? 0 : gst + 1);
+    };
+
     int hsel = 0, wst = 0;
     setup(work);
+    if (GM) {
+        gm_prologue();
+    } else {
 #pragma unroll
     for (int j = 0; j < HPIECES; ++j) issue_h(j, s_begin, Hb0);
     issue_w(s_begin * NTAP, Wb);
     issue_w(s_begin * NTAP + 1, Wb + WBYTES);
+    }
     bool stores_pending = false;
     constexpr int FULL_STORES = (TN / 2 + TN % 2) * TM;
+    bool slab_pending = false;
+    constexpr int SLAB_STORES = TN * TM;
 
     while (true) {
 #pragma unroll
@@ -260,7 +303,7 @@
             for (int a = 0; a < TN; ++a) wf1[a] = bf16x8{0, 0, 0, 0, 0, 0, 0, 0};
         }
 
-        for (int s = s_begin; s < s_end; ++s) {
+        for (int s = s_begin; !GM && s < s_end; ++s) {
             const char* hcur = hsel ? Hb1 : Hb0;
             char* hnext = hsel ? Hb0 : Hb1;
             const bool more = s + 1 < s_end;
@@ -394,7 +437,39 @@
         }
         if (CARRY) mfmas(xf1, wf1);
 
-        if (SC) {
+        if (GM) {
+            for (int t = gt_begin; t < gt_end; ++t) {
+                const bool head = t - gt_begin < NST - 1;
+                const bool sp = stores_pending && head, sl = slab_pending && head;
+                if (t + 1 < gt_end) {
+                    if (sp) wait_vmcnt<7 + FULL_STORES>();
+                    else if (sl) wait_vmcnt<7 + SLAB_STORES>();
+                    else wait_vmcnt<7>();
+                } else {
+                    if (sp) wait_vmcnt<FULL_STORES>();
+                    else if (sl) wait_vmcnt<SLAB_STORES>();
+                    else wait_vmcnt<0>();
+                }
+                __builtin_amdgcn_s_barrier();
+                asm volatile("" ::: "memory");
+                const char* xcur = smem + gst * XSTAGE;
+                const char* wcur = Wb + gst * WBYTES;
+#pragma unroll
+                for (int f = 0; f < TM; ++f) xf0[f] = *(const bf16x8*)(xcur + scfrag + f * 2048);
+#pragma unroll
+                for (int a = 0; a < TN; ++a) wf0[a] = *(const bf16x8*)(wcur + wfrag + a * 2048 + wswz0);
+                __builtin_amdgcn_sched_barrier(0);
+                if (t + NST - 1 < gt_end) stage_gm(t + NST - 1, gst == 0 ? NST - 1 : gst - 1);
+                __builtin_amdgcn_sched_barrier(0);
+#pragma unroll
+                for (int f = 0; f < TM; ++f) xf1[f] = *(const bf16x8*)(xcur + ((scfrag + f * 2048) ^ 64));
+#pragma unroll
+                for (int a = 0; a < TN; ++a) wf1[a] = *(const bf16x8*)(wcur + wfrag + a * 2048 + (wswz0 ^ 64));
+                mfmas(xf0, wf0);
+                mfmas(xf1, wf1);
+                gst = gst == NST - 1 ? 0 : gst + 1;
+            }
+        } else if (SC) {
             const int nsc = (p.Csc1 + p.Csc2) >> 6, nsc1 = p.Csc1 >> 6;
             const int t_begin = (int)((long)nsc * split / p.splitk), t_end = (int)((long)nsc * (split + 1) / p.splitk);
             if (t_begin < t_end) {
@@ -468,7 +543,7 @@
             }
         }
         if (p.splitk == 1) {
-            if (SC == 0 && p.R) {
+            if (SC != 1 && p.R) {
                 u32x2 rr[TN][TM];
 #pragma unroll
                 for (int a = 0; a < TN; ++a) {
@@ -492,7 +567,7 @@
                 for (int a = 0; a < TN; ++a) {
                     const int n = min(en0 + wn * WTN + a * 16 + lq * 4, p.N - 4);
                     f32x4 bv = *(const f32x4*)(p.bias + n);
-                    if (SC == 0 && p.bias2) bv += *(const f32x4*)(p.bias2 + n);
+                    if (SC != 1 && p.bias2) bv += *(const f32x4*)(p.bias2 + n);
 #pragma unroll
                     for (int b = 0; b < TM; ++b) acc[a][b] += bv;
                 }
@@ -502,7 +577,12 @@
         work += gridDim.x;
         const bool more_work = work < nwork;
         const bool wide_ok = (p.ldc & 7) == 0;
-        if (more_work) {
+        if (more_work && GM) {
+            setup(work);
+            gm_prologue();
+            stores_pending = p.splitk == 1 && wide_ok && (em0 + BM <= elim) && (en0 + BN <= p.N);
+            slab_pending = p.splitk > 1 && (em0 + BM <= elim) && (en0 + BN <= p.N);
+        } else if (more_work) {
             setup(work);
             wait_vmcnt<0>();
             char* hb = hsel ? Hb1 : Hb0;
@@ -527,7 +607,7 @@
                 }
             }
         } else {
-            if (!GEN && p.stats) {
+            if (!GEN && p.stats && (!GM || em0 + wm * WTM < Mrows)) {
                 const int r0 = em0 + wm * WTM;
                 const int blk0 = SUB ? ((((r0 >> lgHW) << 2) + ephase) << (lgHW - 6)) + ((r0 & (HWo - 1)) >> 6) : r0 >> 6;
 #pragma unroll
@@ -769,3 +849,56 @@
     SD_CHECK_HIP(hipGetLastError());
     return 0;
 }
+
+bool sd_gemm_wide_applicable(const GemmArgs& a, int epi) {
+    if (epi != 0 || a.dt != 0 || a.out_fp8) return false;
+    if (a.ln_rs || a.rowstats || a.hm_C || a.KV || a.rows_per_batch || a.w_batch_stride) return false;
+    if (a.M <= 0 || a.N <= 0 || a.N % BN) return false;
+    if (a.K1 < 64 || a.K1 % 64 || a.K < a.K1 || (a.K - a.K1) % 64) return false;
+    const long ldx = a.ldx ? a.ldx : a.K1, ldx2 = a.K > a.K1 ? (a.ldx2 ? a.ldx2 : a.K - a.K1) : 0, ldw = a.ldw ? a.ldw : a.K;
+    if (ldx < a.K1 || ldx2 < a.K - a.K1 || ldw < a.K) return false;
+    if ((ldx & 7) || (ldx2 & 7) || (ldw & 7) || (a.ldc & 7) || a.ldc < a.N) return false;
+    if (a.R && ((a.ldr & 7) || a.ldr < a.N)) return false;
+    const long big = 1l << 32;
+    return ((long)a.M + BM) * std::max(ldx, ldx2) * 2 < big && ((long)a.N + BN) * ldw * 2 < big;
+}
+
+int sd_gemm_wide_splitk(int M, int N, int K) {
+    const int tiles = ((M + BM - 1) / BM) * ((N + BN - 1) / BN);
+    if (tiles >= 192) return 1;
+    const int KT = K / 64;
+    const int want = (256 + tiles - 1) / tiles;
+    const int maxs = tiles < 64 ? KT / 18 : KT / 36;
+    int s = want < maxs ? want : maxs;
+    if (s > 8) s = 8;
+    return s < 1 ? 1 : s;
+}
+
+int sd_launch_gemm_wide(const GemmArgs& a0, hipStream_t stream) {
+    SD_REQUIRE(sd_gemm_wide_applicable(a0, 0), "gemm (wide): problem not supported (M=%d N=%d K=%d K1=%d)", a0.M, a0.N, a0.K, a0.K1);
+    SD_REQUIRE(a0.X && a0.W && a0.C && (a0.K1 == a0.K || a0.X2), "gemm (wide): null operand");
+    GemmArgs a = a0;
+    if (a.slab == nullptr || a.splitk < 1) a.splitk = 1;
+    SD_REQUIRE(a.splitk <= a.K / 64, "gemm (wide): splitk %d exceeds the %d K tiles", a.splitk, a.K / 64);
+    SD_REQUIRE(!a.defer_reduce || a.splitk > 1, "gemm (wide): defer_reduce needs split-K (the consumer would read an unwritten slab)");
+    SD_REQUIRE(!a.stats || (a.M % 64 == 0 && a.splitk == 1), "gemm (wide): block statistics need M %% 64 == 0 and no split-K (M=%d splitk=%d)",
+               a.M, a.splitk);
+    a.tiles_m = (a.M + BM - 1) / BM;
+    a.tiles_n = a.N / BN;
+    if (a.ldx == 0) a.ldx = a.K1;
+    if (a.ldx2 == 0) a.ldx2 = a.K - a.K1;
+    if (a.ldw == 0) a.ldw = a.K;
+    a.Xs1 = a.X; a.Xs2 = a.K > a.K1 ? a.X2 : a.X; a.Wsc = a.W; a.ldwsc = a.ldw; a.Csc1 = a.K1; a.Csc2 = a.K - a.K1;
+    a.Cin = 0; a.Hin = a.Win = a.Hout = a.Wout = 1; a.stride = 1; a.up = 0; a.subpix = 0; a.tune = 0;
+    static bool attr_set = false;
+    if (!attr_set) {
+        SD_CHECK_HIP(hipFuncSetAttribute((const void*)conv_halo_kernel<0, 0, 8, 0, 0, 2>, hipFuncAttributeMaxDynamicSharedMemorySize, SMEM));
+        attr_set = true;
+    }
+    int grid = a.tiles_m * a.tiles_n * a.splitk;
+    if (grid > 256) grid = 256;
+    hipLaunchKernelGGL((conv_halo_kernel<0, 0, 8, 0, 0, 2>), dim3(grid), dim3(512), SMEM, stream, a);
+    if (a.splitk > 1 && !a.defer_reduce) sd_launch_splitk_reduce(a, stream);
+    SD_CHECK_HIP(hipGetLastError());
+    return 0;
+}
diff --git a/sonicdiffusionbayeslab_amd/csrc/kernels.h b/sonicdiffusionbayeslab_amd/csrc/kernels.h
--- a/sonicdiffusionbayeslab_amd/csrc/kernels.h
+++ b/sonicdiffusionbayeslab_amd/csrc/kernels.h
@@ -64,6 +64,9 @@
 bool sd_conv_halo_subpix_applicable(const GemmArgs& a);
 int sd_launch_conv3x3_halo(const GemmArgs& a, hipStream_t stream);
 bool sd_conv_halo_shortcut_applicable(const GemmArgs& a);
+bool sd_gemm_wide_applicable(const GemmArgs& a, int epi);
+int sd_gemm_wide_splitk(int M, int N, int K);
+int sd_launch_gemm_wide(const GemmArgs& a, hipStream_t stream);
 
 struct GroupNormArgs {
     const bf16_t* x1 = nullptr; int C1 = 0;
diff --git a/sonicdiffusionbayeslab_amd/csrc/model.h b/sonicdiffusionbayeslab_amd/csrc/model.h
--- a/sonicdiffusionbayeslab_amd/csrc/model.h
+++ b/sonicdiffusionbayeslab_amd/csrc/model.h
@@ -72,6 +72,7 @@
     int asym = 0;
     int hm = 0;
     int qps = 0;
+    int wide = 0;
     int rs = -1, lnrs = -1, lnnp = 0;
     size_t c1 = NOFF;
     size_t wsc = NOFF;
diff --git a/sonicdiffusionbayeslab_amd/csrc/ops.hip b/sonicdiffusionbayeslab_amd/csrc/ops.hip
--- a/sonicdiffusionbayeslab_amd/csrc/ops.hip
+++ b/sonicdiffusionbayeslab_amd/csrc/ops.hip
@@ -479,6 +479,70 @@
     }
     return sd_launch_gemm(a, 0, (hipStream_t)stream);
 }
+static void gemm_wide_args(GemmArgs& a, const void* X, long long ldx, const void* X2, long long ldx2, int K1, const void* W,
+                           const float* bias, const float* bias2, const void* R, long long ldr, void* C, long long ldc, int M, int N,
+                           int K) {
+    a.X = (const bf16_t*)X; a.ldx = ldx; a.X2 = (const bf16_t*)X2; a.ldx2 = ldx2; a.K1 = K1; a.W = (const bf16_t*)W;
+    a.bias = bias; a.bias2 = bias2; a.R = (const bf16_t*)R; a.ldr = ldr; a.C = (bf16_t*)C; a.ldc = ldc; a.M = M; a.N = N; a.K = K;
+    a.zero_page = zero_page();
+}
+extern "C" int sd_op_gemm_wide(void* stream, const void* X, long long ldx, const void* X2, long long ldx2, int K1, const void* W,
+                               const float* bias, const float* bias2, const void* R, long long ldr, void* C, long long ldc,
+                               int M, int N, int K, float* stats) {
+    if (ensure_zero_page()) return -2;
+    GemmArgs a;
+    gemm_wide_args(a, X, ldx, X2, ldx2, K1, W, bias, bias2, R, ldr, C, ldc, M, N, K);
+    SD_REQUIRE(sd_gemm_wide_applicable(a, 0), "sd_op_gemm_wide: problem not supported (M=%d N=%d K=%d K1=%d)", M, N, K, K1);
+    a.stats = stats;
+    a.splitk = stats ? 1 : sd_gemm_wide_splitk(M, N, K);
+    if (splitk_slab(a, "sd_op_gemm_wide")) return -1;
+    return sd_launch_gemm_wide(a, (hipStream_t)stream);
+}
+extern "C" int sd_op_gemm_wide_splitk(int M, int N, int K) {
+    SD_REQUIRE(M > 0 && N > 0 && K > 0, "gemm_wide_splitk: bad arguments");
+    return sd_gemm_wide_splitk(M, N, K);
+}
+extern "C" int sd_op_gemm_wide_applicable(int M, int N, int K, int K1, long long ldx, long long ldx2, long long ldw, long long ldr,
+                                          long long ldc, int epi, int features) {
+    static const float one = 1.f;
+    static bf16_t some;
+    GemmArgs a;
+    a.M = M; a.N = N; a.K = K; a.K1 = K1; a.ldx = ldx; a.ldx2 = ldx2; a.ldw = ldw; a.ldr = ldr; a.ldc = ldc;
+    if (ldr) a.R = &some;
+    if (features & 1) a.ln_rs = &one;
+    if (features & 2) a.rowstats = const_cast<float*>(&one);
+    if (features & 4) { a.hm_C = N / 3; a.KV = &some; }
+    if (features & 8) { a.rows_per_batch = 128; a.w_batch_stride = (long)N * K; }
+    if (features & 16) a.out_fp8 = 1;
+    if (features & 32) a.dt = 1;
+    return sd_gemm_wide_applicable(a, epi) ? 1 : 0;
+}
+extern "C" int sd_op_gemm_wide_groupnorm(void* stream, const void* X, long long ldx, const void* X2, long long ldx2, int K1,
+                                         const void* W, const float* bias, const float* bias2, const void* R, void* C, int M, int N,
+                                         int K, const float* gamma, const float* beta, void* Yn, int B, int groups, float eps,
+                                         int silu, int deferred) {
+    if (ensure_zero_page()) return -2;
+    SD_REQUIRE(B > 0 && M % B == 0, "sd_op_gemm_wide_groupnorm: M=%d is not B=%d samples", M, B);
+    const int HW = M / B;
+    GemmArgs a;
+    gemm_wide_args(a, X, ldx, X2, ldx2, K1, W, bias, bias2, R, N, C, N, M, N, K);
+    SD_REQUIRE(sd_gemm_wide_applicable(a, 0), "sd_op_gemm_wide_groupnorm: problem not supported (M=%d N=%d K=%d K1=%d)", M, N, K, K1);
+    a.splitk = sd_gemm_wide_splitk(M, N, K);
+    const size_t slab_bytes = a.splitk > 1 ? (size_t)a.splitk * M * N * 4 : 0;
+    char* scratch = (char*)op_scratch(slab_bytes + sd_groupnorm_scratch_bytes(B, HW, groups));
+    SD_REQUIRE(scratch, "sd_op_gemm_wide_groupnorm: cannot allocate scratch");
+    if (a.splitk > 1) { a.slab = (float*)scratch; a.defer_reduce = deferred ? 1 : 0; }
+    SD_REQUIRE(!a.defer_reduce || sd_groupnorm_slab_ok(B, HW, N, 0, groups),
+               "sd_op_gemm_wide_groupnorm: the single-launch GroupNorm does not take B=%d HW=%d C=%d groups=%d", B, HW, N, groups);
+    SD_REQUIRE(!deferred || a.defer_reduce, "sd_op_gemm_wide_groupnorm: the deferred form needs split-K (M=%d N=%d K=%d runs unsplit)", M, N, K);
+    if (int rc = sd_launch_gemm_wide(a, (hipStream_t)stream)) return rc;
+    GroupNormArgs g = groupnorm_after_conv(C, N, gamma, beta, Yn, B, HW, groups, eps, silu, (float*)(scratch + slab_bytes), nullptr);
+    if (a.defer_reduce) {
+        g.slab = a.slab; g.splitk = a.splitk; g.sbias = bias; g.sbias2 = bias2; g.sR = (const bf16_t*)R; g.sldr = N;
+        g.x1w = (bf16_t*)C;
+    }
+    return sd_launch_groupnorm(g, (hipStream_t)stream);
+}
 extern "C" int sd_op_gemm_ln(void* stream, const void* X, long long ldx, const void* Wg, const float* c1, const float* c2,
                              const float* rowstats, int parts, float eps, void* C, long long ldc, int M, int N, int K, int epi) {
     if (ensure_zero_page()) return -2;
diff --git a/sonicdiffusionbayeslab_amd/csrc/plan.hip b/sonicdiffusionbayeslab_amd/csrc/plan.hip
--- a/sonicdiffusionbayeslab_amd/csrc/plan.hip
+++ b/sonicdiffusionbayeslab_amd/csrc/plan.hip
@@ -137,13 +137,26 @@
         push(o);
         return o.out;
     }
+    int gemm_wide = getenv("SD_SPLITK") ? 0 : getenv("SD_GEMM_WIDE") ? atoi(getenv("SD_GEMM_WIDE")) : 1;
+    bool wide_gemm(int M, int N, int k1, int k2, int r) const {
+        if (gemm_wide <= 0 || u->kind != 0) return false;
+        if (gemm_wide == 1 && (sd_gemm_splitk(M, N, k1 + k2) <= 1 || sd_gemm_wide_splitk(M, N, k1 + k2) != sd_gemm_splitk(M, N, k1 + k2)))
+            return false;
+        GemmArgs g;
+        g.M = M; g.N = N; g.K = k1 + k2; g.K1 = k1; g.ldx = k1; g.ldx2 = k2; g.ldw = g.K; g.ldc = N;
+        static const bf16_t some = {};
+        if (r >= 0) { g.R = &some; g.ldr = N; }
+        return sd_gemm_wide_applicable(g, 0);
+    }
     int gemm(int x1, int k1, int x2, int k2, int M, int N, const std::string& w, const std::string& b, int r, int epi,
-             bool fq = false, const std::string& oname = "") {
+             bool fq = false, const std::string& oname = "", bool wide = false) {
         Op o; o.kind = OP_GEMM; o.x1 = x1; o.x2 = x2; o.K1 = k1; o.K = k1 + k2; o.Kalg = o.K; o.M = M; o.N = N; o.epi = epi;
         o.b = b.empty() ? NOFF : W(b); o.r = r;
         if (fq) { o.dt = 1; o.K = o.K1 = pad128(k1); o.w = W(w + ".fp8"); o.wsc = W(w + ".scale"); o.xs = xscale(x1); }
         else o.w = W(w);
-        o.splitk = epi ? 1 : sd_gemm_splitk(M, N, o.dt ? o.K / 2 : o.K, o.dt ? 128 : 0);
+        o.wide = wide && !fq && epi == 0 && oname.empty() && wide_gemm(M, N, k1, k2, r);
+        o.splitk = epi ? 1 : o.wide ? sd_gemm_wide_splitk(M, N, o.K)
+                                    : sd_gemm_splitk(M, N, o.dt ? o.K / 2 : o.K, o.dt ? 128 : 0);
         if (o.splitk > 1) o.aux = tensor((size_t)o.splitk * M * N * 4);
         if (!oname.empty()) {
             o.out_fp8 = 1; o.sname = u->act_id(oname, u->s_ff); o.os = u->act_scale[o.sname]; o.Cpad = pad128(N / 2);
@@ -299,7 +312,7 @@
         static const bool merge_off = getenv("SD_FF_MERGE") && atoi(getenv("SD_FF_MERGE")) == 0;
         int out;
         if (!fq && !merge_off) {
-            out = gemm(ff, 4 * C, h2, C, M, C, p + "ff_out.weight", p + "ff_out.bias", x, 0);
+            out = gemm(ff, 4 * C, h2, C, M, C, p + "ff_out.weight", p + "ff_out.bias", x, 0, false, "", true);
         } else {
             int h3 = gemm(ff, 4 * C, -1, 0, M, C, t + "ff.net.2.weight", t + "ff.net.2.bias", h2, 0, fq);
             out = gemm(h3, C, -1, 0, M, C, p + "proj_out.weight", p + "proj_out.bias", x, 0);
diff --git a/sonicdiffusionbayeslab_amd/csrc/unet.hip b/sonicdiffusionbayeslab_amd/csrc/unet.hip
--- a/sonicdiffusionbayeslab_amd/csrc/unet.hip
+++ b/sonicdiffusionbayeslab_amd/csrc/unet.hip
@@ -112,6 +112,7 @@
             if (o.hm) { a.hm_C = o.N / 3; a.hm_tok = o.HW; a.ldc = a.hm_C; a.KV = (bf16_t*)T(o.out) + (long)o.M * a.hm_C; }
             if (o.lnrs >= 0) { a.ln_rs = (const float*)T(o.lnrs); a.ln_np = o.lnnp; a.ln_c1 = (const float*)(wb + o.c1); a.ln_eps = 1e-5f; }
             if (o.lnrs >= 0 && o.s1 >= 0) { a.ln_c1 = (const float*)T(o.s1); a.bias = (const float*)T(o.s2); a.ln_per_sample = 1; }
+            if (o.wide) return sd_launch_gemm_wide(a, stream);
             return sd_launch_gemm(a, o.epi, stream);
         }
         case OP_LN:
```

Result: no change. 11.30 images/s (-0.0%).
